# gyuhyun-lee/offline_raytracer

Measured on AMD Instinct MI355X. Metric: Mpaths/s, higher is better.
Workload: dtype f32; 1 GPU; c3_bunny_room.scn (69451 triangles) 1920x1080 1024spp rr0.8, CHUNK policy chunk=64, one frame sharded in 8x8 blocks over 1 GPU(s); width=1920, height=1080, spp=1024, gather=none (1 GPU): un-permute kernel only, gather_fallback=False, launch=single process, workspace_bytes_per_rank=398131200

## Files before the change

offline_raytracer_amd/csrc/ort_device.h:

```cpp
#ifndef ORT_DEVICE_H
#define ORT_DEVICE_H

#include <hip/hip_runtime.h>
#include <stdint.h>

#include "ort_detmath.h"

namespace ortd {

#ifdef ORT_HOST_SIM
#define ORT_D static inline
#else
#define ORT_D __device__ __forceinline__
#endif

struct V3 { float x, y, z; };

constexpr float kPi = 3.14159265358979323846264338327950288419716939937510582097494459230f;
constexpr float kEuler = 2.71828182845904523536028747135266249f;
constexpr float kHitTMin = 0.000001f;
constexpr float kRoughness = 0.01f;
constexpr float kEps = 0.0001f;

ORT_D V3 mk(float x, float y, float z) { V3 r; r.x = x; r.y = y; r.z = z; return r; }
ORT_D V3 add(V3 a, V3 b) { return mk(a.x + b.x, a.y + b.y, a.z + b.z); }
ORT_D V3 sub(V3 a, V3 b) { return mk(a.x - b.x, a.y - b.y, a.z - b.z); }
ORT_D V3 neg(V3 a) { return mk(-a.x, -a.y, -a.z); }
ORT_D V3 scale(float s, V3 a) { return mk(s * a.x, s * a.y, s * a.z); }
ORT_D V3 divs(V3 a, float s) { return mk(a.x / s, a.y / s, a.z / s); }
ORT_D V3 had(V3 a, V3 b) { return mk(a.x * b.x, a.y * b.y, a.z * b.z); }
ORT_D float dot(V3 a, V3 b) { return a.x * b.x + a.y * b.y + a.z * b.z; }
ORT_D float len2(V3 a) { return a.x * a.x + a.y * a.y + a.z * a.z; }
ORT_D float len(V3 a) { return __builtin_sqrtf(a.x * a.x + a.y * a.y + a.z * a.z); }
ORT_D V3 cross(V3 a, V3 b) {
    return mk(a.y * b.z - b.y * a.z, b.x * a.z - a.x * b.z, a.x * b.y - b.x * a.y);
}
ORT_D float absr(float v) { if (v <= 0.0f) v *= -1.0f; return v; }
ORT_D float sq(float v) { return v * v; }
ORT_D bool ceq(float a, float b) { float d = a - b; return d >= -0.000001f && d < 0.000001f; }
ORT_D float sgn(float a) { return (a >= 0.0f) ? 1.0f : -1.0f; }
ORT_D float rmin(float a, float b) { return (a < b) ? a : b; }
ORT_D float rmax(float a, float b) { return (a > b) ? a : b; }
ORT_D V3 normalize(V3 a) {
    float l = len(a);
    if (__builtin_expect(!ceq(l, 0.0f), 1)) return divs(a, l);
    return mk(0, 0, 0);
}
ORT_D bool isnan3(V3 v) { return (v.x != v.x) || (v.y != v.y) || (v.z != v.z); }
ORT_D bool isinf1(float v) { return (om_f32_bits(v) & 0x7fffffffu) == 0x7f800000u; }
ORT_D bool isinf3(V3 v) { return isinf1(v.x) || isinf1(v.y) || isinf1(v.z); }

ORT_D void rng_step(uint32_t &s) { s ^= s << 13; s ^= s >> 17; s ^= s >> 5; }
ORT_D float rng_01(uint32_t &s) { rng_step(s); return (float)s / 4294967296.0f; }
ORT_D float rng_between(uint32_t &s, float lo, float hi) { rng_step(s); return lo + (hi - lo) * rng_01(s); }

ORT_D uint32_t fmix32(uint32_t h) {
    h ^= h >> 16; h *= 0x85ebca6bu; h ^= h >> 13; h *= 0xc2b2ae35u; h ^= h >> 16;
    return h;
}
ORT_D uint32_t job_seed(uint32_t master, uint32_t job) {
    uint32_t h = fmix32(master ^ (job * 2654435761u));
    return h ? h : 1u;
}

struct Mat {
    V3 kd; float ior;
    V3 ks; uint32_t is_light;
    V3 kt; float pd_c;
    V3 emit; float ps_c;
    V3 ed; float pt_c;
};
ORT_D Mat load_mat(const float4 *mats, uint32_t index) {
    const float4 *p = mats + 5u * index;
    float4 a = p[0], b = p[1], c = p[2], d = p[3], e = p[4];
    Mat m;
    m.kd = mk(a.x, a.y, a.z); m.ior = a.w;
    m.ks = mk(b.x, b.y, b.z); m.is_light = om_f32_bits(b.w);
    m.kt = mk(c.x, c.y, c.z); m.pd_c = c.w;
    m.emit = mk(d.x, d.y, d.z); m.ps_c = d.w;
    m.ed = mk(e.x, e.y, e.z); m.pt_c = e.w;
    return m;
}
ORT_D Mat make_mat(V3 kd, V3 ks, V3 kt, float ior) {
    Mat m;
    m.kd = kd; m.ks = ks; m.kt = kt; m.ior = ior; m.is_light = 0; m.emit = mk(0, 0, 0);
    float a = len(kd), b = len(ks), c = len(kt);
    float s = a + b + c;
    m.pd_c = a / s; m.ps_c = b / s; m.pt_c = c / s;
    m.ed = divs(kd, kPi);
// ... 102 lines not shown
        float r = radicand(m, wo, bn.n);
        if (r >= 0.0f) {
            float n_m = dot(N, m), wi_m = dot(wi, m), wo_m = dot(wo, m);
            float denom = sq(bn.no * wo_m + bn.no * wo_m);
            if (!ceq(denom, 0.0f)) {
                float D = ggx_d(N, m, rough);
                pt = D * absr(n_m) * sq(bn.no) * absr(wi_m) / denom;
            }
        }
    }
    return pd_c * pd + ps_c * ps + pt_c * pt;
}

ORT_D float pdf_eval_scattering(V3 N, V3 wi, V3 wo, const Mat &mt, float rough, float dist, float rr, V3 &f) {
    const float wi_n = dot(wi, N), wo_n = dot(wo, N);
    const bool has_ks = len2(mt.ks) > 0.0f, has_kt = len2(mt.kt) > 0.0f;
    V3 H = mk(0, 0, 0);
    float wi_h = 0.0f, D_h = 0.0f, ps = 0.0f;
    if (mt.ps_c > 0.0f || has_ks) {
        H = scale(sgn(wi_n), normalize(add(wo, wi)));
        wi_h = dot(wi, H);
        const float denom = (4.0f * absr(wi_h));
        const bool pdf_needs = mt.ps_c > 0.0f && !ceq(denom, 0.0f);
        if (pdf_needs || (has_ks && wi_h > 0.0f)) D_h = ggx_d(N, H, rough);
        if (pdf_needs) ps = D_h * absr(dot(N, H)) / denom;
    }
    Beer bn; bn.ni = bn.no = bn.n = 0.0f;
    V3 m = mk(0, 0, 0);
    float r = -1.0f, D_m = 0.0f, wi_m = 0.0f, wo_m = 0.0f, pt = ps;
    if (mt.pt_c > 0.0f || has_kt) {
        bn = beer(N, wo, mt.ior);
        m = normalize(neg(add(scale(bn.ni, wi), scale(bn.no, wo))));
        r = radicand(m, wo, bn.n);
        if (!(r < 0.0f)) {
            wi_m = dot(wi, m); wo_m = dot(wo, m);
            D_m = ggx_d(N, m, rough);
        }
        if (r >= 0.0f && mt.pt_c > 0.0f) {
            const float denom = sq(bn.no * wo_m + bn.no * wo_m);
            if (!ceq(denom, 0.0f)) pt = D_m * absr(dot(N, m)) * sq(bn.no) * absr(wi_m) / denom;
        }
    }
    const float pd = absr(wi_n) / kPi;
    const float p = (mt.pd_c * pd + mt.ps_c * ps + mt.pt_c * pt) * rr;
    if (!(p > 0.000001f)) return p;
    V3 Es = mk(0, 0, 0), Et = mk(0, 0, 0);
    if (has_ks && wi_h > 0.0f) {
        V3 F = fresnel(mt.ks, wi_h);
        float G = geom(wi, N, H, rough) * geom(wo, N, H, rough);
        Es = scale((D_h * G) / (4.0f * absr(wi_n) * absr(wo_n)), F);
    }
    if (has_kt) {
        V3 At = mk(1, 1, 1);
        if (wo_n < 0) {
            At.x = ort_powf(kEuler, dist * ort_logf(mt.kt.x));
            At.y = ort_powf(kEuler, dist * ort_logf(mt.kt.y));
            At.z = ort_powf(kEuler, dist * ort_logf(mt.kt.z));
        }
        if (r < 0.0f) {
            if (has_ks) Et = had(At, Es);
        } else {
            V3 F = sub(mk(1, 1, 1), fresnel(mt.ks, wi_m));
            float G = geom(wi, N, m, rough) * geom(wo, N, m, rough);
            float denom = (absr(wi_n) * absr(wo_n) * sq(bn.ni * wi_m + bn.no * wo_m));
            if (!ceq(denom, 0.0f)) {
                V3 nom = scale(D_m * G * absr(wi_m) * absr(wo_m) * sq(bn.no), F);
                Et = had(At, divs(nom, denom));
            }
        }
    }
    f = scale(absr(wi_n), add(add(mt.ed, Es), Et));
    return p;
}

ORT_D V3 sample_lobe_n(V3 N, float c, float cos_phi, float sin_phi) {
    float s = __builtin_sqrtf(1.0f - c * c);
    V3 K = mk(s * cos_phi, s * sin_phi, c);
    if (absr(N.z - 1.0f) < 0.0001f) return K;
    if (absr(N.z + 1.0f) < 0.0001f) return mk(K.x, -K.y, -K.z);
    V3 B = normalize(mk(-N.y, N.x, 0));
    V3 C = cross(N, B);
    return add(add(scale(K.x, B), scale(K.y, C)), scale(K.z, N));
}
ORT_D V3 sample_lobe(V3 N, float c, float phi) { return sample_lobe_n(normalize(N), c, ort_cosf(phi), ort_sinf(phi)); }

struct BrdfDraw { float c, phi, choice; };
template <bool DIFFUSE_SCENE = false>
ORT_D BrdfDraw sample_brdf_draw(uint32_t &rng, float rough, const Mat &mt) {
    float e0 = rng_01(rng), e1 = rng_01(rng);
    BrdfDraw d;
    d.choice = rng_01(rng);
    d.phi = 2.0f * kPi * e1;
    const bool diffuse_lobe = d.choice < mt.pd_c;
    if (DIFFUSE_SCENE ? __builtin_expect(diffuse_lobe, 1) : diffuse_lobe) d.c = __builtin_sqrtf(e0);
    else d.c = ort_cosf(ort_atan2f(rough * __builtin_sqrtf(e0), __builtin_sqrtf(1.0f - e0)));
    return d;
}
template <bool NORMALIZED = true, bool DIFFUSE_SCENE = false>
ORT_D V3 sample_brdf_finish(V3 N, V3 Nn, V3 wo, const Mat &mt, BrdfDraw d, float cos_phi, float sin_phi, bool &is_trans) {
    float pd_c = mt.pd_c, ps_c = mt.ps_c;
    V3 wi;
    is_trans = false;
    V3 m = sample_lobe_n(Nn, d.c, cos_phi, sin_phi);
    const bool diffuse_lobe = d.choice < pd_c;
    if (DIFFUSE_SCENE ? __builtin_expect(diffuse_lobe, 1) : diffuse_lobe) {
        wi = m;
    } else {
        bool refract = !(d.choice >= pd_c && d.choice < pd_c + ps_c);
        Beer bn;
        float r = 0.0f;
        if (refract) {
            bn = beer(N, wo, mt.ior);
            r = radicand(m, wo, bn.n);
            refract = !(r < 0.0f);
        }
        if (!refract) {
            wi = sub(scale(2.0f * absr(dot(wo, m)), m), wo);
        } else {
            wi = sub(scale(bn.n * dot(wo, m) - sgn(dot(wo, N)) * __builtin_sqrtf(r), m), scale(bn.n, wo));
            is_trans = true;
        }
    }
    return NORMALIZED ? normalize(wi) : wi;
}
ORT_D V3 sample_brdf(uint32_t &rng, V3 N, V3 wo, float rough, const Mat &mt, bool &is_trans) {
    BrdfDraw d = sample_brdf_draw(rng, rough, mt);
    return sample_brdf_finish(N, normalize(N), wo, mt, d, ort_cosf(d.phi), ort_sinf(d.phi), is_trans);
}

ORT_D float hit_triangle(V3 v0, V3 e1, V3 e2, V3 o, V3 d) {
    V3 pv = cross(d, e2);
    float det = dot(pv, e1);
    if (!(det <= -0.000001f || det >= 0.000001f)) return -1.0f;
    V3 T = sub(o, v0);
    float u = dot(pv, T) / det;
    if (!(u >= 0.0f)) return -1.0f;
    V3 a = cross(T, e1);
    float v = dot(a, d) / det;
    if (!(v >= 0.0f && u + v <= 1.0f)) return -1.0f;
    float t = dot(a, e2) / det;
    if (!(t >= kHitTMin)) return -1.0f;
    return t;
}

ORT_D float hit_sphere(V3 c, float rad, V3 o, V3 d, V3 &n, bool &tangent) {
    float ht = -1.0f;
    tangent = false;
    V3 rel = sub(o, c);
    float a = dot(d, d), b = dot(d, rel), cc = dot(rel, rel) - rad * rad;
    float root = b * b - a * cc;
    const float tol = 0.00001f;
    if (root >= tol) {
        float sr = __builtin_sqrtf(root);
        float tn = (-b - sr) / a, tp = (-b + sr) / a;
        float t = (tn < 0.0f) ? tp : tn;
        if (t > kHitTMin) {
            ht = t;
            n = scale(1.0f, sub(add(o, scale(ht, d)), c));
        }
    } else if (__builtin_expect(root < tol && root > -tol, 0)) {
        float t = (-b) / (2 * a);
        if (t > kHitTMin) {
            ht = t;
            n = sub(add(o, scale(ht, d)), c);
            tangent = true;
        }
    }
    return ht;
}

ORT_D float hit_aab(V3 lo, V3 hi, V3 o, V3 inv, V3 &n) {
    float ht = -1.0f;
    V3 t0 = had(sub(lo, o), inv), t1 = had(sub(hi, o), inv);
    V3 tmin = mk(rmin(t0.x, t1.x), rmin(t0.y, t1.y), rmin(t0.z, t1.z));
    V3 tmax = mk(rmax(t0.x, t1.x), rmax(t0.y, t1.y), rmax(t0.z, t1.z));
    float max_of_min = rmax(rmax(tmin.x, tmin.y), tmin.z);
    float min_of_max = rmin(rmin(tmax.x, tmax.y), tmax.z);
    if (min_of_max >= max_of_min) {
        float tx = t0.x, ty = t0.y, tz = t0.z;
        float sx = -1.0f, sy = -1.0f, sz = -1.0f;
        if (tx > t1.x) { tx = t1.x; sx = 1.0f; }
        if (ty > t1.y) { ty = t1.y; sy = 1.0f; }
        if (tz > t1.z) { tz = t1.z; sz = 1.0f; }
        float best = tx;
        V3 bn = mk(sx, 0, 0);
        if (best < ty) { best = ty; bn = mk(0, sy, 0); }
// ... 75 lines not shown
```

offline_raytracer_amd/csrc/ort_kernels.hip:

```cpp
#include <algorithm>
#include <memory>
#include <type_traits>

#include "ort_lane.h"
#include "ort_plan.h"
#include "ort_setup.h"

#ifndef ORT_HOST_SIM
void ort_launch_w5(int diffuse, unsigned int grid, void *stream, const void *sv_bytes, const void *hot_bytes);
void ort_w5_layout(size_t sizes[3]);
void ort_launch_radiance_adaptive(int counters, int diffuse, int tabs, unsigned int grid, void *stream, const void *sv_bytes, const void *hot_bytes);
void ort_adaptive_layout(size_t sizes[3]);
void ort_launch_render_adaptive(int counters, int diffuse, int tabs, unsigned int grid, void *stream, const void *sv_bytes, const void *hot_bytes);
void ort_render_adaptive_layout(size_t sizes[3]);

namespace ort {

using namespace ortd;

static_assert(kPlanBlock == (uint32_t)kBlock && kPlanLdsStack == (uint32_t)kLdsStack && kPlanStashVecs == kStashVecs && kPlanCapL == kCapL &&
              kPlanCapR == kCapR && (int)PLAN_JOBS_EXPLICIT == (int)JOBS_EXPLICIT &&
              (int)PLAN_JOBS_PIXEL == (int)JOBS_PIXEL && (int)PLAN_JOBS_CHUNK == (int)JOBS_CHUNK,
              "ort_plan.h counts with the lane code's limits");

#define ORT_HIP(call)                                                                          \
    do {                                                                                       \
        hipError_t e_ = (call);                                                                \
        if (e_ != hipSuccess) {                                                                \
            *err = std::string(#call) + ": " + hipGetErrorString(e_);                          \
            return ORT_ERR_HIP;                                                                \
        }                                                                                      \
    } while (0)

struct DevBuf {
    void *p = nullptr;
    size_t bytes = 0;
    DevBuf() = default;
    DevBuf(DevBuf &&o) noexcept : p(o.p), bytes(o.bytes) { o.p = nullptr; o.bytes = 0; }
    DevBuf &operator=(DevBuf &&o) noexcept { std::swap(p, o.p); std::swap(bytes, o.bytes); return *this; }
    ~DevBuf() { if (p) (void)hipFree(p); }
    int ensure(size_t need, std::string *err) {
        if (bytes >= need && p) return ORT_OK;
        if (p) ORT_HIP(hipFree(p));
        p = nullptr;
        bytes = 0;
        ORT_HIP(hipMalloc(&p, need ? need : 16));
        bytes = need;
        return ORT_OK;
    }
    template <typename T> T *as() const { return (T *)p; }
};

struct DeviceScene {
    explicit DeviceScene(int device_index) : device(device_index) {}
    ~DeviceScene() {
        (void)hipSetDevice(device);
        if (h_active) (void)hipHostFree(h_active);
        for (hipEvent_t ev : {ev0, ev1, ev_done})
            if (ev) (void)hipEventDestroy(ev);
    }
    const int device;
    Knobs knobs;
    DevBuf nodes, tris, spheres, boxes, cyls, materials;
    DevBuf nodes4;
    DevBuf prim_info;
    uint32_t info_box = 0, info_cyl = 0, info_sphere = 0;
    DevBuf light_is_sphere;
    DevBuf tab;
    DevBuf cold;
    DevBuf rv_dev;
    DevBuf view_tab;
    std::vector<float> view_tab_host;
    uint32_t tab_flags = 0;
    uint32_t light_count = 0;
    bool diffuse_only = false;
    DevBuf ref_nodes, ref_recs, chain_boxes;
    DevBuf tri_order, sphere_order, box_order, cyl_order;
    DevBuf bfs_pool, bfs_locks;
    uint32_t bfs_queue_cap = 0, bfs_queue_count = 0;
    unsigned int max_blocks = 0;
    DevBuf ctrl_buf;
    unsigned long long *ctrl() const { return ctrl_buf.as<unsigned long long>(); }
    DevBuf partial, staging, jobs, states;
    hipEvent_t ev0 = nullptr, ev1 = nullptr;
    hipEvent_t ev_done = nullptr;
    bool inflight = false;
    int cu_count = 0;
    DevBuf stash;
    DevBuf drain;
    DevBuf wf_mem;
    unsigned long long *h_active = nullptr;
    DevBuf prim_src;
    float scene_lo[3] = {0, 0, 0}, scene_hi[3] = {0, 0, 0};
    bool scene_box_known = false;
    DevBuf query_stage[6];
};

int device_count(int *n, std::string *err) {
    int c = 0;
    hipError_t e = hipGetDeviceCount(&c);
    if (e != hipSuccess) { *n = 0; *err = std::string("hipGetDeviceCount: ") + hipGetErrorString(e); return ORT_ERR_NO_DEVICE; }
    *n = c;
    return ORT_OK;
}

template <typename T>
static int upload_vec(const std::vector<T> &v, DevBuf *dst, std::string *err) {
    size_t bytes = v.size() * sizeof(T);
    int rc = dst->ensure(bytes, err);
    if (rc) return rc;
    if (bytes) ORT_HIP(hipMemcpy(dst->p, v.data(), bytes, hipMemcpyHostToDevice));
    return ORT_OK;
}

void device_release(Scene *scene) {
    delete scene->dev;
    scene->dev = nullptr;
}

int device_upload(Scene *scene, int device, std::string *err) {
    int n = 0;
    int rc = device_count(&n, err);
    if (rc != ORT_OK) return rc;
    if (n <= 0) { *err = "no HIP device visible"; return ORT_ERR_NO_DEVICE; }
    if (device < 0 || device >= n) { *err = "device index out of range"; return ORT_ERR_INVALID; }
    device_release(scene);
    ORT_HIP(hipSetDevice(device));
    std::unique_ptr<DeviceScene> owner(new DeviceScene(device));
    DeviceScene *d = owner.get();
    const Tree &t = scene->tree;
    if ((rc = upload_vec(t.nodes, &d->nodes, err))) return rc;
    if (!t.nodes4.empty() && 3u * t.max_depth4 <= (uint32_t)(kLdsStack - 4 + kSpillStack))
        if ((rc = upload_vec(t.nodes4, &d->nodes4, err))) return rc;
    if ((rc = upload_vec(t.tris, &d->tris, err))) return rc;
    if ((rc = upload_vec(t.spheres, &d->spheres, err))) return rc;
    if ((rc = upload_vec(t.boxes, &d->boxes, err))) return rc;
    if ((rc = upload_vec(t.cyls, &d->cyls, err))) return rc;
    {
        std::vector<PrimInfo> info;
        build_prim_info(t, scene->ref, info, d->info_box, d->info_cyl, d->info_sphere);
        if ((rc = upload_vec(info, &d->prim_info, err))) return rc;
    }
    const std::vector<DevMaterial> mats = dev_materials(*scene);
    if ((rc = upload_vec(mats, &d->materials, err))) return rc;
    d->diffuse_only = true;
    for (size_t i = 1; i < mats.size(); ++i) {
        const DevMaterial &dm = mats[i];
        if (dm.is_light) continue;
        const float ks2 = dm.specular[0] * dm.specular[0] + dm.specular[1] * dm.specular[1] + dm.specular[2] * dm.specular[2];
        const float kt2 = dm.transmission[0] * dm.transmission[0] + dm.transmission[1] * dm.transmission[1] + dm.transmission[2] * dm.transmission[2];
        if (ks2 > 0.0f || kt2 > 0.0f || dm.ps_c > 0.0f || dm.pt_c > 0.0f) d->diffuse_only = false;
    }
    const std::vector<uint32_t> lis = light_sphere_flags(*scene);
    d->light_count = (uint32_t)lis.size();
    if ((rc = upload_vec(lis, &d->light_is_sphere, err))) return rc;
    {
        std::vector<F4> tab;
        d->tab_flags = pack_lds_tables(t, mats, lis, tab);
        if ((rc = upload_vec(tab, &d->tab, err))) return rc;
    }
    const RefTree &rt = scene->ref;
    if ((rc = upload_vec(rt.nodes, &d->ref_nodes, err))) return rc;
    if ((rc = upload_vec(rt.recs, &d->ref_recs, err))) return rc;
    if ((rc = upload_vec(rt.chain_boxes, &d->chain_boxes, err))) return rc;
    if ((rc = upload_vec(rt.tri_order, &d->tri_order, err))) return rc;
    if ((rc = upload_vec(rt.sphere_order, &d->sphere_order, err))) return rc;
    if ((rc = upload_vec(rt.box_order, &d->box_order, err))) return rc;
    if ((rc = upload_vec(rt.cyl_order, &d->cyl_order, err))) return rc;
    if ((rc = d->ctrl_buf.ensure(128 * sizeof(unsigned long long), err))) return rc;
    ORT_HIP(hipMemset(d->ctrl(), 0, 128 * sizeof(unsigned long long)));
    ORT_HIP(hipEventCreate(&d->ev0));
    ORT_HIP(hipEventCreate(&d->ev1));
    ORT_HIP(hipEventCreateWithFlags(&d->ev_done, hipEventDisableTiming));
    hipDeviceProp_t prop;
    ORT_HIP(hipGetDeviceProperties(&prop, device));
    d->cu_count = prop.multiProcessorCount;
    d->knobs = read_knobs();
    d->max_blocks = upload_max_blocks(d->cu_count, d->knobs);
    d->bfs_queue_cap = (uint32_t)rt.nodes.size() + 8u;
    size_t fit = kBfsPoolBytes / ((size_t)d->bfs_queue_cap * sizeof(uint32_t));
    d->bfs_queue_count = (uint32_t)(fit < 16 ? 16 : (fit > kBfsPoolQueues ? kBfsPoolQueues : fit));
    if ((rc = d->bfs_pool.ensure((size_t)d->bfs_queue_count * d->bfs_queue_cap * sizeof(uint32_t), err))) return rc;
    if ((rc = d->bfs_locks.ensure((size_t)d->bfs_queue_count * kBfsLockStride * sizeof(uint32_t), err))) return rc;
    ORT_HIP(hipMemset(d->bfs_locks.p, 0, d->bfs_locks.bytes));
    ORT_HIP(hipHostMalloc((void **)&d->h_active, sizeof(unsigned long long)));
    {
        SceneCold cold{};
        cold.ref_nodes = d->ref_nodes.as<const float4>(); cold.ref_recs = d->ref_recs.as<const uint32_t>();
        cold.tri_order = d->tri_order.as<const uint32_t>(); cold.sphere_order = d->sphere_order.as<const uint32_t>();
        cold.box_order = d->box_order.as<const uint32_t>(); cold.cyl_order = d->cyl_order.as<const uint32_t>();
        cold.bfs_pool = d->bfs_pool.as<uint32_t>(); cold.bfs_locks = d->bfs_locks.as<uint32_t>();
        cold.bfs_queue_cap = d->bfs_queue_cap; cold.bfs_queue_count = d->bfs_queue_count;
        cold.fallback_counters = d->ctrl() + 6;
        if ((rc = d->rv_dev.ensure(sizeof(RenderView), err))) return rc;
        if ((rc = d->cold.ensure(sizeof(SceneCold), err))) return rc;
        ORT_HIP(hipMemcpy(d->cold.p, &cold, sizeof(SceneCold), hipMemcpyHostToDevice));
    }
    scene->dev = owner.release();
    return ORT_OK;
}

int device_unit_eval(int device, const void *records, uint32_t n, float *out, std::string *err) {
    int count = 0;
    int rc = device_count(&count, err);
    if (rc != ORT_OK) return rc;
    if (device < 0 || device >= count) { *err = "no such HIP device"; return ORT_ERR_NO_DEVICE; }
    ORT_HIP(hipSetDevice(device));
    DevBuf d_rec, d_out;
    if ((rc = d_rec.ensure((size_t)n * 100u + 16, err)) || (rc = d_out.ensure((size_t)n * 32u + 16, err))) return rc;
    ORT_HIP(hipMemcpy(d_rec.p, records, (size_t)n * 100u, hipMemcpyHostToDevice));
    if (n) hipLaunchKernelGGL(unit_eval, dim3((n + 63) / 64), dim3(64), 0, 0, d_rec.as<const uint32_t>(), n, d_out.as<float>());
    ORT_HIP(hipGetLastError());
    ORT_HIP(hipMemcpy(out, d_out.p, (size_t)n * 32u, hipMemcpyDeviceToHost));
    return ORT_OK;
}

template <bool COUNTERS>
static int launch_wavefront(DeviceScene *d, const LaunchPlan &, const SceneView &sv, const RenderView &rvf, const RenderHot &rv, hipStream_t stream, std::string *err) {
    const uint32_t kMaxSlots = 1u << 21;
    unsigned long long want = rvf.job_count < kMaxSlots ? rvf.job_count : kMaxSlots;
    uint32_t S = (uint32_t)((want + kBlock - 1) / kBlock) * kBlock;
    if (S == 0) S = kBlock;
    const size_t per_slot = 16 + 8 + 16 + 4 + 16 + 16 + 16 + 16 + 4;
    size_t need = (size_t)S * per_slot + 4096;
    int rc = d->wf_mem.ensure(need, err);
    if (rc) return rc;
    WfView wf{};
    wf.slots = S;
    char *base = d->wf_mem.as<char>();
    auto carve = [&](size_t bytes) { char *p = base; base += (bytes + 255) & ~(size_t)255; return p; };
    wf.active = (unsigned long long *)carve(256);
    wf.od0 = (float4 *)carve((size_t)S * 16); wf.hit0 = (float4 *)carve((size_t)S * 16);
    wf.p0 = (float4 *)carve((size_t)S * 16); wf.p1 = (float4 *)carve((size_t)S * 16); wf.p2 = (float4 *)carve((size_t)S * 16);
    wf.p3 = (uint4 *)carve((size_t)S * 16);
    wf.od1 = (float2 *)carve((size_t)S * 8);
    wf.hitp = (uint32_t *)carve((size_t)S * 4); wf.flags = (uint32_t *)carve((size_t)S * 4);
    if ((size_t)(base - d->wf_mem.as<char>()) > d->wf_mem.bytes) { *err = "internal: wavefront state carve overflow"; return ORT_ERR_INVALID; }

    unsigned int blocks = S / kBlock;
    unsigned int grid = blocks < d->max_blocks * 2u ? blocks : d->max_blocks * 2u;
    hipLaunchKernelGGL(wf_init, dim3(blocks), dim3(kBlock), 0, stream, wf);
    ORT_HIP(hipGetLastError());
    const int batch = 32;
    for (;;) {
        for (int it = 0; it < batch; ++it) {
            int last = (it == batch - 1);
            if (last) ORT_HIP(hipMemsetAsync(wf.active, 0, sizeof(unsigned long long), stream));
            hipLaunchKernelGGL(wf_shade<COUNTERS>, dim3(grid), dim3(kBlock), 0, stream, sv, rv, wf, last);
            hipLaunchKernelGGL(wf_trace<COUNTERS>, dim3(grid), dim3(kBlock), 0, stream, sv, rv, wf);
        }
        ORT_HIP(hipGetLastError());
        ORT_HIP(hipMemcpyAsync(d->h_active, wf.active, sizeof(unsigned long long), hipMemcpyDeviceToHost, stream));
        ORT_HIP(hipStreamSynchronize(stream));
        if (*d->h_active == 0ull) break;
    }
    return ORT_OK;
}

static int launch_five_waves(DeviceScene *, const LaunchPlan &pl, const SceneView &sv, const RenderView &, const RenderHot &hot, hipStream_t stream, std::string *) {
    ort_launch_w5(pl.diffuse ? 1 : 0, pl.grid, (void *)stream, &sv, &hot);
// ... 25 lines not shown
    loop<true, false, false>(), loop<true, false, true>(), loop<true, true, false>(), loop<true, true, true>(),
    loop<false, false, true, true, true>(), loop<false, true, true, true, true>(), loop<true, false, true, false, true>(),
    views<false, false, false>(), views<false, false, true, true>(), views<false, true, false>(), views<false, true, true, true>(),
    views<true, false, false>(), views<true, false, true>(),
    exchange<false, false>(), exchange<false, true>(), exchange<true, true>(),
    five(false), five(true),
    adaptive(false, false, false), adaptive(false, false, true), adaptive(false, true, false), adaptive(false, true, true),
    adaptive(true, false, false), adaptive(true, false, true), adaptive(true, true, false), adaptive(true, true, true),
};
constexpr bool launchers_match(size_t i = 0) { return i == kBuiltKernelCount || (kLaunchers[i].variant == kBuiltKernels[i] && launchers_match(i + 1)); }
static_assert(sizeof(kLaunchers) / sizeof(kLaunchers[0]) == kBuiltKernelCount && launchers_match(),
              "kLaunchers holds the entries of kBuiltKernels (ort_plan.h), all of them, in its order");

static int launch_path_tracer(DeviceScene *d, const LaunchPlan &pl, const SceneView &sv, const RenderView &rv, const RenderHot &hot, hipStream_t stream, std::string *err) {
    const size_t i = built_index(plan_variant(pl));
    if (i == kBuiltKernelCount) { *err = "internal: no kernel is built for this launch plan"; return ORT_ERR_INTERNAL; }
    if (kLaunchers[i].host) return kLaunchers[i].host(d, pl, sv, rv, hot, stream, err);
    hipLaunchKernelGGL(kLaunchers[i].kernel, dim3(pl.grid), dim3(kBlock), 0, stream, sv, hot);
    return ORT_OK;
}

static int settle_inflight(DeviceScene *d, std::string *err, const char *what = "the previous render on this scene overflowed a reference-order fallback queue") {
    if (!d->inflight) return ORT_OK;
    ORT_HIP(hipEventSynchronize(d->ev_done));
    d->inflight = false;
    unsigned long long ovf = 0;
    ORT_HIP(hipMemcpy(&ovf, d->ctrl() + 7, sizeof(ovf), hipMemcpyDeviceToHost));
    if (ovf) { *err = what; return ORT_ERR_UNSUPPORTED; }
    return ORT_OK;
}

static int reset_ctrl(DeviceScene *d, RenderView *rv, hipStream_t stream, std::string *err) {
    rv->next_job = d->ctrl();
    rv->counters = d->ctrl() + 1;
    ORT_HIP(hipMemsetAsync(d->ctrl(), 0, 128 * sizeof(unsigned long long), stream));
    return ORT_OK;
}
static int upload_view(DeviceScene *d, const RenderView &rv, bool timed, hipStream_t stream, RenderHot *hot, std::string *err) {
    ORT_HIP(hipMemcpyAsync(d->rv_dev.p, &rv, sizeof(RenderView), hipMemcpyHostToDevice, stream));
    *hot = render_hot<RenderHot>(rv, d->rv_dev.p);
    if (timed) ORT_HIP(hipEventRecord(d->ev0, stream));
    return ORT_OK;
}
static int end_kernels(DeviceScene *d, bool timed, hipStream_t stream, std::string *err) {
    ORT_HIP(hipGetLastError());
    if (timed) ORT_HIP(hipEventRecord(d->ev1, stream));
    return ORT_OK;
}
static int mark_inflight(DeviceScene *d, hipStream_t stream, std::string *err) {
    ORT_HIP(hipEventRecord(d->ev_done, stream));
    d->inflight = true;
    return ORT_OK;
}

static int add_launch_stats(const DeviceScene *d, bool counters, bool paths, ort_stats *stats, std::string *err) {
    float ms = 0;
    ORT_HIP(hipEventElapsedTime(&ms, d->ev0, d->ev1));
    unsigned long long c[6];
    ORT_HIP(hipMemcpy(c, d->ctrl() + 1, sizeof(c), hipMemcpyDeviceToHost));
    stats->kernel_ms += ms;
    stats->fallback_rays += c[5];
    if (counters) { stats->rays += c[1]; stats->node_tests += c[2]; stats->tri_tests += c[3]; stats->analytic_tests += c[4]; }
    if (counters && paths) stats->paths += c[0];
    return ORT_OK;
}

static SceneView scene_view(Scene *scene, DeviceScene *d) {
    SceneView sv{};
    sv.nodes = d->nodes.as<const float4>(); sv.tris = d->tris.as<const float4>();
    sv.spheres = d->spheres.as<const float4>(); sv.boxes = d->boxes.as<const float4>(); sv.cyls = d->cyls.as<const float4>();
    sv.prim_info = d->prim_info.as<const PrimInfo>();
    sv.info_box = d->info_box; sv.info_cyl = d->info_cyl; sv.info_sphere = d->info_sphere;
    sv.materials = d->materials.as<const float4>();
    sv.light_is_sphere = d->light_is_sphere.as<const uint32_t>();
    sv.tab_src = d->tab.as<const float4>();
    sv.tab_flags = d->tab_flags;
    sv.light_count = d->light_count;
    sv.pro_boxes = scene->tree.pro_boxes;
    sv.pro_spheres = scene->tree.pro_spheres;
    sv.pro_cyls = scene->tree.pro_cyls;
    sv.chain_boxes = d->chain_boxes.as<const float4>();
    if (getenv("ORT_KNOBS_LIVE")) { const int keep = d->knobs.blocks_per_cu; d->knobs = read_knobs(); d->knobs.blocks_per_cu = keep; }
    sv.force_fallback_mask = d->knobs.force_fallback_mask;
    sv.cold = (const ORT_CONSTANT_AS SceneCold *)d->cold.p;
    return sv;
}

static size_t fast_tree_bytes(const Scene *scene) { return scene->tree.nodes.size() * sizeof(DevNode) + scene->tree.tris.size() * sizeof(DevTri); }

static SceneTraits scene_traits(const Scene *scene, const DeviceScene *d) {
    SceneTraits t;
    t.diffuse_only = d->diffuse_only;
    t.tab_flags = d->tab_flags;
    t.fast_tree_bytes = fast_tree_bytes(scene);
    t.sah_cost = scene->tree.sah_cost;
    t.has_wide = d->nodes4.p != nullptr;
    t.cu_count = d->cu_count;
    t.max_blocks = d->max_blocks;
    return t;
}

static int print_fallback_diag(const DeviceScene *d, const LaunchPlan &pl, std::string *err) {
    unsigned long long fb[2], dg[3];
    ORT_HIP(hipMemcpy(fb, d->ctrl() + 6, sizeof(fb), hipMemcpyDeviceToHost));
    ORT_HIP(hipMemcpy(dg, d->ctrl() + 6 + kDiagFallback, sizeof(dg), hipMemcpyDeviceToHost));
    fprintf(stderr, "fallback: %llu rays traversed again without their first winner, %llu re-cast exactly (%llu octree nodes enqueued, %llu busy queues met)\n",
            dg[1], fb[0], dg[0], dg[2]);
    fprintf(stderr, "issue order: %s\n", pl.block_major ? "block-major" : "chunk-major");
    return ORT_OK;
}

static int print_drain_diag(const DeviceScene *d, const LaunchPlan &pl, std::string *err) {
    std::vector<unsigned long long> t((size_t)pl.grid * (kBlock / 64));
    ORT_HIP(hipMemcpy(t.data(), d->drain.p, t.size() * sizeof(unsigned long long), hipMemcpyDeviceToHost));
    unsigned long long last = 0;
    for (unsigned long long v : t) last = v > last ? v : last;
    const double tick_ms = 1e-5;
    const double marks[] = {0.25, 0.5, 1, 2, 3, 5, 8, 12, 20};
    fprintf(stderr, "drain: of %zu waves, still running before the end of the launch:", t.size());
    for (double m : marks) {
        size_t n = 0;
        for (unsigned long long v : t) n += (double)(last - v) * tick_ms < m ? 1 : 0;
        fprintf(stderr, "  %g ms: %zu", m, n);
    }
    fprintf(stderr, "\n");
    return ORT_OK;
}

static int print_util_diag(const DeviceScene *d, std::string *err) {
    static const char *names[8] = {"node visit", "leaf visit", "traverse outer iteration", "shade call", "  of which lanes with a finished ray",
                                   "produce_ray pass", "  bounce draw", "  sin/cos + ray setup"};
    unsigned long long u[16];
    ORT_HIP(hipMemcpy(u, d->ctrl() + 8, sizeof(u), hipMemcpyDeviceToHost));
    for (int k = 0; k < 8; ++k)
        fprintf(stderr, "util %-40s wave-events %14llu  mean active lanes %6.2f\n", names[k], u[2 * k],
                u[2 * k] ? (double)u[2 * k + 1] / (double)u[2 * k] : 0.0);
    static const char *pnames[10] = {"resolve_hit (chain check)", "hit processing + bounce draw", "pixel / job / new sample", "sin/cos + normalise + ray setup",
                                    "1/d + analytic prologue", "descend loop", "leaf", "pt_lane loop top (after traverse)",
                                    "produce_ray entry (after resolve)", "traverse loop top"};
    unsigned long long ph[30];
    ORT_HIP(hipMemcpy(ph, d->ctrl() + 8 + 32, sizeof(ph), hipMemcpyDeviceToHost));
    double total = 0;
    for (int k = 0; k < 10; ++k) total += (double)ph[3 * k];
    for (int k = 0; k < 10; ++k)
        fprintf(stderr, "phase %-36s share %5.1f %%  cycles/mark %8.1f  marks %12llu  lanes at mark %5.1f\n", pnames[k],
                total > 0 ? 100.0 * (double)ph[3 * k] / total : 0.0, ph[3 * k + 1] ? (double)ph[3 * k] / (double)ph[3 * k + 1] : 0.0,
                ph[3 * k + 1], ph[3 * k + 1] ? (double)ph[3 * k + 2] / (double)ph[3 * k + 1] : 0.0);
    return ORT_OK;
}

static bool same_layout(void (*unit_layout)(size_t *)) {
    size_t s[3];
    unit_layout(s);
    return s[0] == sizeof(SceneView) && s[1] == sizeof(RenderHot) && s[2] == sizeof(RenderView);
}

int device_render(Scene *scene, const ort_render_params *p, const RenderCall &c, void *out_rgb, void *out_spp, void *out_m2, void *states, std::string *err) {
    DeviceScene *d = scene->dev;
    if (!d) { *err = "scene is not uploaded to a device (ort_scene_upload)"; return ORT_ERR_NO_DEVICE; }
    ORT_HIP(hipSetDevice(d->device));
    if (c.ad && !same_layout(ort_render_adaptive_layout)) { *err = "internal: the adaptive render kernels were built with other argument layouts"; return ORT_ERR_INTERNAL; }
    hipStream_t stream = (hipStream_t)c.stream;
    const uint32_t view_count = c.views ? c.view_count : 1u;
    int rc;
    if ((rc = settle_inflight(d, err))) return rc;

// ... 252 lines not shown
```

offline_raytracer_amd/csrc/ort_lane.h:

```cpp
#ifndef ORT_LANE_H
#define ORT_LANE_H

#include <hip/hip_runtime.h>

#include <math.h>
#include <stdio.h>
#include <stdlib.h>
#include <string.h>

#include <algorithm>
#include <string>
#include <vector>

#include "ort_device.h"
#include "ort_scene.h"
#include "ort_setup.h"

#ifdef ORT_W5_TU
#define ORT_NS ort_w5
#elif defined(ORT_ADAPTIVE_TU)
#define ORT_NS ort_ad
#elif defined(ORT_RENDER_ADAPTIVE_TU)
#define ORT_NS ort_ra
#else
#define ORT_NS ort
#endif

namespace ORT_NS {

using namespace ort;
using namespace ortd;

constexpr int kBlock = 256;
#ifndef ORT_LDS_STACK
#define ORT_LDS_STACK 24
#endif
constexpr int kLdsStack = ORT_LDS_STACK;
#ifndef ORT_SPILL_STACK
#define ORT_SPILL_STACK 40
#endif
constexpr int kSpillStack = ORT_SPILL_STACK;
static_assert(kLdsStack - 4 + kSpillStack >= (int)kTreeDepthBudget, "the re-traversal of resolve_hit must hold a tree of kTreeDepthBudget levels");
constexpr uint32_t kBfsPoolQueues = 1024;
constexpr size_t kBfsPoolBytes = 1024u << 20;
constexpr int kDiagFallback = 106;
constexpr uint32_t kBfsLockStride = 32;


#ifdef ORT_HOST_SIM
#define ORT_CONSTANT_AS
#else
#define ORT_CONSTANT_AS __attribute__((address_space(4)))
#endif
struct SceneCold {
    const float4 *ref_nodes;
    const uint32_t *ref_recs;
    const uint32_t *tri_order, *sphere_order, *box_order, *cyl_order;
    uint32_t *bfs_pool;
    uint32_t *bfs_locks;
    uint32_t bfs_queue_cap, bfs_queue_count;
    unsigned long long *fallback_counters;
};

struct PrimInfo { uint32_t chain, mat; };

struct SceneView {
    const float4 *tab_src;
    uint32_t tab_flags;
    const float4 *nodes;
    const float4 *tris;
    const float4 *spheres;
    const float4 *boxes;
    const float4 *cyls;
    const PrimInfo *prim_info;
    uint32_t info_box, info_cyl, info_sphere;
    const float4 *materials;
    const uint32_t *light_is_sphere;
    uint32_t light_count;
    uint32_t pro_boxes, pro_spheres, pro_cyls;
    float cam[12];
    const float4 *chain_boxes;
    const ORT_CONSTANT_AS SceneCold *cold;
    unsigned long long *util;
    uint32_t force_fallback_mask;
};

inline void build_prim_info(const Tree &t, const RefTree &rt, std::vector<PrimInfo> &out, uint32_t &info_box, uint32_t &info_cyl, uint32_t &info_sphere) {
    info_box = (uint32_t)t.tri_mat.size();
    info_cyl = info_box + (uint32_t)t.box_mat.size();
    info_sphere = info_cyl + (uint32_t)t.cyl_mat.size();
    out.assign((size_t)info_sphere + t.sphere_mat.size(), PrimInfo{0u, 0u});
    auto fill = [&out](uint32_t base, const std::vector<uint32_t> &chain, const std::vector<uint32_t> &mat) {
        for (size_t i = 0; i < mat.size(); ++i) out[base + i] = PrimInfo{i < chain.size() ? chain[i] : 0u, mat[i]};
    };
    fill(0u, rt.tri_chain, t.tri_mat);
    fill(info_box, rt.box_chain, t.box_mat);
    fill(info_cyl, rt.cyl_chain, t.cyl_mat);
    fill(info_sphere, rt.sphere_chain, t.sphere_mat);
}

enum : int { JOBS_EXPLICIT = 0, JOBS_PIXEL = 1, JOBS_CHUNK = 2 };

struct RenderView {
    int mode;
    const ort_tile_job *jobs;
    uint32_t *final_states;
    unsigned long long job_count;
    int W, H, x0, y0, x1, y1;
    uint32_t seed, spp, chunk, nchunks;
    float rr;
    int refill_below;
    int descend_below;
    uint32_t shard_index, shard_count, blocks_w, my_blocks;
    uint32_t block_x0, block_y0;
    float *out;
    float *partial;
    int packed_out;
    unsigned long long *next_job;
    unsigned long long *counters;
    float4 *stash;
    uint32_t stash_wave_f4;
    uint32_t capL, capR;
    uint32_t long_min;
    uint32_t long_refill;
    uint32_t park_min;
    uint32_t inflight_cap;
    uint32_t block_major;
    unsigned long long endgame_from;
    uint32_t job_batch;
    unsigned long long batch_until;
    unsigned long long *drain;
    const float4 *views;
    unsigned long long view_jobs;
    uint32_t view_count;
    const float2 *rays;
    const uint32_t *seeds;
    uint32_t ray_tree_spheres, ray_tree_quadrics, ray_tree_boxes;
    float ray_lo[3], ray_hi[3];
    uint32_t ad_min_spp, ad_check_every;
    float ad_tolerance, ad_floor;
    uint32_t *ad_spp;
    float *ad_m2;
};


struct RenderHot {
    int mode, W, H;
    float rr;
    int refill_below, descend_below;
    const ORT_CONSTANT_AS RenderView *c;
};

struct WfView {
    uint32_t slots;
    float4 *od0;
    float2 *od1;
    float4 *hit0;
    uint32_t *hitp;
    float4 *p0;
    float4 *p1;
    float4 *p2;
    uint4 *p3;
    uint32_t *flags;
    unsigned long long *active;
};

enum : int { PS_NEED_JOB = 0, PS_PIXEL = 1, PS_SAMPLE = 2, PS_HIT = 3, PS_DONE = 4 };

#ifdef ORT_HOST_SIM
#define ORT_BALLOT(p) ((p) ? 1ull : 0ull)
#define ORT_POPC64(m) __builtin_popcountll(m)
#define ORT_NEXT_JOB(p) __atomic_fetch_add((p), 1ull, __ATOMIC_RELAXED)
#define ORT_COUNT(p, v) ((void)__atomic_fetch_add((p), (v), __ATOMIC_RELAXED))
#define ORT_TRY_LOCK(p) (*(p) == 0u ? (*(p) = 1u, true) : false)
#define ORT_PEEK(p) (*(p))
#define ORT_BACKOFF()
#define ORT_UNLOCK(p) (*(p) = 0u)
#define ORT_FENCE()
#define ORT_FFS64(m) __builtin_ffsll((long long)(m))
#define ORT_LANE() 0
#define ORT_UTIL(sv, k, pred)
// ... 45 lines not shown
    } while (0)
#endif

#ifndef ORT_HOST_SIM
__shared__ unsigned long long g_lds_prof[96 + 4];
#endif

struct Prof { unsigned long long t = 0; bool on = false; };

#ifndef ORT_DESCEND_SHIFT
#define ORT_DESCEND_SHIFT 2
#endif

#define ORT_RARE(x) __builtin_expect(!!(x), 0)
#if defined(ORT_HOST_SIM) && defined(ORT_CHAIN_STATS)
extern unsigned long long g_cs[4][16];
#define ORT_STAT(row, col) (g_cs[row][col]++)
#else
#define ORT_STAT(row, col) ((void)0)
#endif
constexpr uint32_t kNoPrim = 0xffffffffu;
constexpr uint32_t kTraversalDone = 0xffffffffu;

ORT_D uint32_t prim_order(const SceneView &sv, uint32_t kind, uint32_t slot) {
    return (kind == PRIM_TRI) ? sv.cold->tri_order[slot] : (kind == PRIM_SPHERE) ? sv.cold->sphere_order[slot]
         : (kind == PRIM_BOX) ? sv.cold->box_order[slot] : sv.cold->cyl_order[slot];
}

template <bool COUNTERS, bool EXACT_ORDER, bool FINITE_RAY = false, bool FROM_TAB = false>
ORT_D void test_prim(const SceneView &sv, uint32_t kind, uint32_t slot, V3 org, V3 dir, V3 inv_d, float &best_t, V3 &hit_n,
                     uint32_t &hit_prim, float &phantom_t, float &runner_t, unsigned long long &c_tris, unsigned long long &c_analytic,
                     uint32_t excl = 0xffffffffu, const float4 *rec = nullptr ) {
    float t;
    V3 n = mk(0, 0, 0);
    bool tangent = false;
    if (!EXACT_ORDER && ((kind << 28) | slot) == excl) return;
    if (kind == PRIM_TRI) {
        const float4 *tp = sv.tris + 3u * slot;
        float4 a = tp[0], b = tp[1], c = tp[2];
        if (COUNTERS) c_tris++;
        t = hit_triangle(mk(a.x, a.y, a.z), mk(a.w, b.x, b.y), mk(b.z, b.w, c.x), org, dir);
        n = mk(c.y, c.z, c.w);
    } else if (kind == PRIM_SPHERE) {
        float4 s;
        if (FROM_TAB) s = rec[0]; else s = sv.spheres[slot];
        if (COUNTERS) c_analytic++;
        t = hit_sphere(mk(s.x, s.y, s.z), s.w, org, dir, n, tangent);
    } else if (kind == PRIM_BOX) {
        float4 lo, hi;
        if (FROM_TAB) { lo = rec[0]; hi = rec[1]; } else { lo = sv.boxes[2u * slot]; hi = sv.boxes[2u * slot + 1u]; }
        if (COUNTERS) c_analytic++;
        t = FINITE_RAY ? hit_aab_finite(mk(lo.x, lo.y, lo.z), mk(hi.x, hi.y, hi.z), org, inv_d, n)
                       : hit_aab(mk(lo.x, lo.y, lo.z), mk(hi.x, hi.y, hi.z), org, inv_d, n);
    } else {
        float4 a, b, c, d;
        if (FROM_TAB) { a = rec[0]; b = rec[1]; c = rec[2]; d = rec[3]; }
        else { const float4 *cp = sv.cyls + 4u * slot; a = cp[0]; b = cp[1]; c = cp[2]; d = cp[3]; }
        if (COUNTERS) c_analytic++;
        t = hit_cylinder(mk(a.x, a.y, a.z), a.w, mk(b.x, b.y, b.z), mk(b.w, c.x, c.y), mk(c.z, c.w, d.x), d.y, org, dir, n);
    }
    if (!EXACT_ORDER && tangent) {
        phantom_t = fminf(phantom_t, t);
        return;
    }
    bool take = (t >= kHitTMin && t < best_t);
    if (!EXACT_ORDER && t == best_t && t >= kHitTMin && hit_prim != kNoPrim) {
        take = prim_order(sv, kind, slot) < prim_order(sv, hit_prim >> 28, hit_prim & 0x00ffffffu);
    }
    if (!EXACT_ORDER && t >= kHitTMin) runner_t = fminf(runner_t, take ? best_t : t);
    if (take) {
        best_t = t;
        hit_n = n;
        hit_prim = (kind << 28) | slot;
    }
}

enum : int { CH_ADMIT = 0, CH_REJECT = 1, CH_UNKNOWN = 2 };

ORT_D uint32_t info_index(const SceneView &sv, uint32_t prim) {
    const uint32_t kind = prim >> 28, slot = prim & 0x00ffffffu;
    return slot + ((kind == PRIM_TRI) ? 0u : (kind == PRIM_BOX) ? sv.info_box : (kind == PRIM_CYL) ? sv.info_cyl : sv.info_sphere);
}

template <int BLOCK>
ORT_D void announce_winner(const SceneView &sv, uint32_t prim, uint32_t *lds_stack, int tid) {
    if (prim == kNoPrim) return;
    const PrimInfo *p = sv.prim_info + info_index(sv, prim);
#ifdef ORT_HOST_SIM
    lds_stack[tid] = p->chain;
    lds_stack[BLOCK + tid] = p->mat;
#else
    const uint32_t dst = (uint32_t)__builtin_amdgcn_readfirstlane((int)(uint32_t)(uintptr_t)(lds_stack + (tid & ~63)));
    const uint32_t *q = &p->mat;
    unsigned keep;
    asm volatile("s_mov_b32 %0, m0\n\ts_mov_b32 m0, %3\n\ts_nop 0\n\tglobal_load_lds_dword %1, off\n\t"
                 "s_add_u32 m0, %3, %4\n\ts_nop 0\n\tglobal_load_lds_dword %2, off\n\ts_mov_b32 m0, %0"
                 : "=&s"(keep) : "v"(p), "v"(q), "s"(dst), "n"(BLOCK * 4) : "scc");
#endif
}

template <int BLOCK>
ORT_D void announced_info(const uint32_t *lds_stack, int tid, uint32_t &chain, uint32_t &mat) {
#ifndef ORT_HOST_SIM
    asm volatile("s_waitcnt vmcnt(0)" ::: "memory");
#endif
    chain = lds_stack[tid];
    mat = lds_stack[BLOCK + tid];
}
ORT_D int ref_node_verdict(V3 lo, V3 hi, V3 org, V3 inv_d, float t_hit, float t_other, float &gap) {
    if ((org.x >= lo.x && org.x < hi.x) && (org.y >= lo.y && org.y < hi.y) && (org.z >= lo.z && org.z < hi.z)) return CH_ADMIT;
    const float t = hit_aab_t(lo, hi, org, inv_d);
    if (!(t >= kHitTMin)) return CH_REJECT;
    if (t <= t_hit || (t < t_other && t < t_hit * 1.0001f)) return CH_ADMIT;
    gap = fmaxf(gap, t);
    return CH_UNKNOWN;
}

ORT_D int chain_verdict_full(const SceneView &sv, uint32_t first, uint32_t len, V3 org, V3 inv_d, float t_hit, float t_other, float &gap) {
    int verdict = CH_ADMIT;
    for (uint32_t base = 0; base < len; base += 4u) {
        float4 lo[4], hi[4];
#pragma unroll
        for (uint32_t k = 0; k < 4u; ++k) {
            uint32_t i = base + k;
            i = (i < len) ? i : (len - 1u);
            lo[k] = sv.chain_boxes[2u * (first + i)];
            hi[k] = sv.chain_boxes[2u * (first + i) + 1u];
        }
#pragma unroll
        for (uint32_t k = 0; k < 4u; ++k) {
            const int v = ref_node_verdict(mk(lo[k].x, lo[k].y, lo[k].z), mk(hi[k].x, hi[k].y, hi[k].z), org, inv_d, t_hit, t_other, gap);
            verdict = (v == CH_REJECT || verdict == CH_REJECT) ? CH_REJECT : (v == CH_UNKNOWN ? CH_UNKNOWN : verdict);
        }
        if (verdict == CH_REJECT) break;
    }
    return verdict;
}

ORT_D bool in_rect_half_open(float4 lo, float4 hi, V3 org) {
    return (org.x >= lo.x && org.x < hi.x) && (org.y >= lo.y && org.y < hi.y) && (org.z >= lo.z && org.z < hi.z);
}

constexpr uint32_t kChainNested = 0x08000000u;
#if defined(ORT_HOST_SIM) && defined(ORT_CHAIN_CROSSCHECK)
static unsigned long long g_chain_crosschecks = 0;
#endif
ORT_D int chain_verdict(const SceneView &sv, uint32_t word, V3 org, V3 inv_d, float t_hit, float t_other, float &gap) {
#ifdef ORT_MEASURE_NO_CHAIN
    gap = 0.0f;
    return CH_ADMIT;
#endif
    const uint32_t len = word >> 28, first = word & 0x07ffffffu;
    gap = 0.0f;
    if (len == 0u) return CH_ADMIT;
    const bool finite = (om_f32_bits(inv_d.x) & 0x7fffffffu) < 0x7f800000u && (om_f32_bits(inv_d.y) & 0x7fffffffu) < 0x7f800000u &&
                        (om_f32_bits(inv_d.z) & 0x7fffffffu) < 0x7f800000u;
    if (ORT_RARE(!(word & kChainNested) || !finite)) return chain_verdict_full(sv, first, len, org, inv_d, t_hit, t_other, gap);
    const float4 dlo = sv.chain_boxes[2u * first], dhi = sv.chain_boxes[2u * first + 1u];
    float4 jlo = dlo, jhi = dhi;
    bool found = false;
#ifndef ORT_CHAIN_ROUND
#define ORT_CHAIN_ROUND 2
#endif
    if (len >= 2u) {
        const uint32_t it = len - 1u, it1 = (len >= 3u) ? len - 2u : 1u;
        const float4 plo = sv.chain_boxes[2u * (first + 1u)], phi = sv.chain_boxes[2u * (first + 1u) + 1u];
        const float4 tlo = sv.chain_boxes[2u * (first + it)], thi = sv.chain_boxes[2u * (first + it) + 1u];
        const float4 ulo = sv.chain_boxes[2u * (first + it1)], uhi = sv.chain_boxes[2u * (first + it1) + 1u];
        if (!in_rect_half_open(plo, phi, org)) {
            found = true;
            if (!in_rect_half_open(tlo, thi, org)) { jlo = tlo; jhi = thi; }
            else if (!in_rect_half_open(ulo, uhi, org)) { jlo = ulo; jhi = uhi; }
            else {
                jlo = plo; jhi = phi;
                bool hit = false;
                for (int32_t top = (int32_t)len - 3; ORT_RARE(!hit && top >= 2); top -= ORT_CHAIN_ROUND) {
                    float4 lo[ORT_CHAIN_ROUND], hi[ORT_CHAIN_ROUND];
#pragma unroll
                    for (int32_t k = 0; k < ORT_CHAIN_ROUND; ++k) {
                        int32_t i = top - k;
                        i = (i > 2) ? i : 2;
                        lo[k] = sv.chain_boxes[2u * (first + (uint32_t)i)];
                        hi[k] = sv.chain_boxes[2u * (first + (uint32_t)i) + 1u];
                    }
#pragma unroll
                    for (int32_t k = 0; k < ORT_CHAIN_ROUND; ++k) {
                        const bool outside = !in_rect_half_open(lo[k], hi[k], org);
                        if (!hit && outside) { jlo = lo[k]; jhi = hi[k]; hit = true; }
                    }
                }
            }
        }
    }
#if defined(ORT_HOST_SIM) && defined(ORT_CHAIN_STATS)
    { int jj = -1; for (int32_t i = (int32_t)len - 1; i >= 1; --i) if (!in_rect_half_open(sv.chain_boxes[2u*(first+i)], sv.chain_boxes[2u*(first+i)+1u], org)) { jj = (int)len - 1 - i; break; }
      g_cs[0][len]++; g_cs[1][jj < 0 ? 15 : jj]++; }
#endif
    int verdict = CH_ADMIT;
    if (found && !(hit_aab_t(mk(jlo.x, jlo.y, jlo.z), mk(jhi.x, jhi.y, jhi.z), org, inv_d) >= kHitTMin)) verdict = CH_REJECT;
    else verdict = ref_node_verdict(mk(dlo.x, dlo.y, dlo.z), mk(dhi.x, dhi.y, dhi.z), org, inv_d, t_hit, t_other, gap);
#if defined(ORT_HOST_SIM) && defined(ORT_CHAIN_CROSSCHECK)
    {
        float g2 = 0.0f;
        if (verdict != chain_verdict_full(sv, first, len, org, inv_d, t_hit, t_other, g2)) { fprintf(stderr, "chain shortcut disagrees with the full walk\n"); abort(); }
        g_chain_crosschecks++;
    }
#endif
    return verdict;
}

template <bool COUNTERS>
ORT_D bool ref_raycast_bfs(const SceneView &sv, V3 org, V3 dir, V3 inv_d, uint32_t *queue, float &best_t, V3 &hit_n,
                           uint32_t &hit_prim, unsigned long long &c_nodes, unsigned long long &c_tris,
                           unsigned long long &c_analytic) {
    best_t = 3.402823466e+38f;
    hit_n = mk(0, 0, 0);
    hit_prim = kNoPrim;
    float unused = 0;
    uint32_t head = 0, tail = 0;
    bool ok = true;
    const uint32_t cap = sv.cold->bfs_queue_cap;
    queue[tail++] = 0;
    while (head != tail) {
        uint32_t node = queue[head++];
        const float4 *np = sv.cold->ref_nodes + 3u * node;
        float4 a = np[0], b = np[1], c = np[2];
        int32_t first_child = (int32_t)om_f32_bits(a.w);
        uint32_t rec_first = om_f32_bits(b.w), rec_count = om_f32_bits(c.x);
        for (uint32_t r = 0; r < rec_count; ++r) {
            uint32_t rec = sv.cold->ref_recs[rec_first + r];
            test_prim<COUNTERS, true>(sv, rec >> 28, rec & 0x00ffffffu, org, dir, inv_d, best_t, hit_n, hit_prim, unused, unused, c_tris, c_analytic);
        }
        if (first_child >= 0) {
            for (uint32_t k = 0; k < 8u; ++k) {
                uint32_t ci = (uint32_t)first_child + k;
                const float4 *cp = sv.cold->ref_nodes + 3u * ci;
                float4 ca = cp[0], cb = cp[1], cc = cp[2];
                uint32_t flags = om_f32_bits(cc.y);
                bool leaf_with_records = (flags & 3u) == 3u;
                bool has_children = (int32_t)om_f32_bits(ca.w) >= 0;
                if (!(leaf_with_records || has_children)) continue;
                V3 lo = mk(ca.x, ca.y, ca.z), hi = mk(cb.x, cb.y, cb.z);
                bool add = (org.x >= lo.x && org.x < hi.x) && (org.y >= lo.y && org.y < hi.y) && (org.z >= lo.z && org.z < hi.z);
                if (!add) {
                    float t = hit_aab_t(lo, hi, org, inv_d);
                    if (COUNTERS) c_nodes++;
                    add = (t >= kHitTMin && t < best_t);
                }
                if (add) {
                    if (tail >= cap) { ok = false; continue; }
                    queue[tail++] = ci;
                }
            }
        }
    }
    ORT_COUNT(sv.cold->fallback_counters + kDiagFallback, (unsigned long long)tail);
    return ok;
}

struct Counters {
    unsigned long long paths = 0, rays = 0, nodes = 0, tris = 0, analytic = 0;
};

struct PathState {
    int ps = PS_NEED_JOB;
    uint32_t rng = 0, job_index = 0;
    uint32_t pxy = 0;
    uint32_t jxx = 0;
    uint32_t jyp = 0;
    uint32_t spp = 0, sample = 0;
    V3 color, org, dir, wo, weight;
    bool primary = true;
};

struct AdaptState {
    float q = 0;
    uint32_t next = 0;
};

struct HitState {
    float best_t = 0;
    V3 hit_n;
    uint32_t hit_prim = kNoPrim;
    float phantom_t = 0;
    float runner_t = 0;
    uint32_t hit_mat = 0;
};

ORT_D size_t packed_index(const RenderHot &rv, uint32_t x, uint32_t y) {
    const uint32_t blk = ((y >> 3) - rv.c->block_y0) * rv.c->blocks_w + ((x >> 3) - rv.c->block_x0);
    return (size_t)((blk - rv.c->shard_index) / rv.c->shard_count) * 64u + ((y & 7u) << 3) + (x & 7u);
}
ORT_D float *pixel_ptr(const RenderHot &rv, uint32_t plane, uint32_t x, uint32_t y) {
    if (rv.mode == JOBS_CHUNK) return rv.c->partial + ((size_t)plane * rv.c->my_blocks * 64u + packed_index(rv, x, y)) * 3u;
    if (rv.c->packed_out) return rv.c->out + packed_index(rv, x, y) * 3u;
    return rv.c->out + 3u * ((size_t)y * (size_t)rv.W + (size_t)x);
}

ORT_D float *view_pixel_ptr(const RenderHot &rv, uint32_t view, uint32_t plane, uint32_t x, uint32_t y) {
    if (rv.mode == JOBS_CHUNK) return rv.c->partial + (((size_t)view * rv.c->nchunks + plane) * rv.c->my_blocks * 64u + packed_index(rv, x, y)) * 3u;
    return rv.c->out + 3u * (((size_t)view * (size_t)rv.H + (size_t)y) * (size_t)rv.W + (size_t)x);
}

struct Trav {
    uint32_t cur = 0;
    int sp = 0;
    V3 inv_d;
};

ORT_D void reset_hit(HitState &h, float best_t) {
    h.best_t = best_t;
    h.hit_n = mk(0, 0, 0);
    h.hit_prim = kNoPrim;
    h.phantom_t = __builtin_inff();
    h.runner_t = __builtin_inff();
}

template <bool COUNTERS, bool TABS, bool HAS_EXCL = false>
ORT_D void prologue_tests(const SceneView &sv, const float4 *tab, V3 org, V3 dir, V3 inv_d, HitState &h, Counters &c, uint32_t excl = kNoPrim) {
    const float4 *pb = nullptr, *ps = nullptr, *pc = nullptr;
    if (TABS) { pb = tab + kTabPro; ps = pb + 2u * sv.pro_boxes; pc = ps + sv.pro_spheres; }
#ifndef ORT_PROLOGUE_DEFER
#define ORT_PROLOGUE_DEFER 1
#endif
    if (!ORT_PROLOGUE_DEFER && ORT_BALLOT(!all_finite6(org, inv_d)) == 0ull) {
        for (uint32_t i = 0; i < sv.pro_boxes; ++i)
            test_prim<COUNTERS, false, true, TABS>(sv, PRIM_BOX, i, org, dir, inv_d, h.best_t, h.hit_n, h.hit_prim, h.phantom_t, h.runner_t, c.tris, c.analytic, excl, TABS ? pb + 2u * i : nullptr);
    } else
    if (ORT_BALLOT(!all_finite6(org, inv_d)) == 0ull) {
        for (uint32_t i = 0; i < sv.pro_boxes; ++i) {
            float4 lo, hi;
            if (TABS) { lo = pb[2u * i]; hi = pb[2u * i + 1u]; } else { lo = sv.boxes[2u * i]; hi = sv.boxes[2u * i + 1u]; }
            const uint32_t prim = ((uint32_t)PRIM_BOX << 28) | i;
            if (COUNTERS && (!HAS_EXCL || prim != excl)) c.analytic++;
            float t = hit_aab_t_finite(mk(lo.x, lo.y, lo.z), mk(hi.x, hi.y, hi.z), org, inv_d);
            if (HAS_EXCL && ORT_RARE(prim == excl)) t = -1.0f;
            bool take = (t >= kHitTMin && t < h.best_t);
            if (ORT_RARE(t == h.best_t && t >= kHitTMin && h.hit_prim != kNoPrim))
                take = prim_order(sv, PRIM_BOX, i) < prim_order(sv, h.hit_prim >> 28, h.hit_prim & 0x00ffffffu);
            if (t >= kHitTMin) h.runner_t = fminf(h.runner_t, take ? h.best_t : t);
            if (take) { h.best_t = t; h.hit_prim = prim; }
        }
        if ((h.hit_prim >> 28) == PRIM_BOX && h.hit_prim != kNoPrim) {
            const uint32_t i = h.hit_prim & 0x00ffffffu;
            float4 lo, hi;
            if (TABS) { lo = pb[2u * i]; hi = pb[2u * i + 1u]; } else { lo = sv.boxes[2u * i]; hi = sv.boxes[2u * i + 1u]; }
            V3 n = mk(0, 0, 0);
            (void)hit_aab_finite(mk(lo.x, lo.y, lo.z), mk(hi.x, hi.y, hi.z), org, inv_d, n);
            h.hit_n = n;
        }
    } else {
        for (uint32_t i = 0; i < sv.pro_boxes; ++i)
            test_prim<COUNTERS, false, false, TABS>(sv, PRIM_BOX, i, org, dir, inv_d, h.best_t, h.hit_n, h.hit_prim, h.phantom_t, h.runner_t, c.tris, c.analytic, excl, TABS ? pb + 2u * i : nullptr);
    }
    for (uint32_t i = 0; i < sv.pro_spheres; ++i)
        test_prim<COUNTERS, false, false, TABS>(sv, PRIM_SPHERE, i, org, dir, inv_d, h.best_t, h.hit_n, h.hit_prim, h.phantom_t, h.runner_t, c.tris, c.analytic, excl, TABS ? ps + i : nullptr);
    for (uint32_t i = 0; i < sv.pro_cyls; ++i)
        test_prim<COUNTERS, false, false, TABS>(sv, PRIM_CYL, i, org, dir, inv_d, h.best_t, h.hit_n, h.hit_prim, h.phantom_t, h.runner_t, c.tris, c.analytic, excl, TABS ? pc + 4u * i : nullptr);
}

#ifndef ORT_HOST_SIM
ORT_D float wave_bcast(float v, int lane) { return om_bits_f32((uint32_t)__builtin_amdgcn_readlane((int)om_f32_bits(v), lane)); }
ORT_D uint32_t wave_bcast(uint32_t v, int lane) { return (uint32_t)__builtin_amdgcn_readlane((int)v, lane); }
ORT_D uint32_t rank_in(unsigned long long mask) {
    return __builtin_amdgcn_mbcnt_hi((uint32_t)(mask >> 32), __builtin_amdgcn_mbcnt_lo((uint32_t)mask, 0u));
}

template <bool COUNTERS>
ORT_D bool ref_raycast_bfs_wave(const SceneView &sv, const int leader, V3 org_l, V3 dir_l, V3 inv_l, uint32_t *queue, float &out_t, V3 &out_n,
                                uint32_t &out_prim, unsigned long long &c_nodes, unsigned long long &c_tris, unsigned long long &c_analytic) {
// ... 121 lines not shown
        const bool ok = ref_raycast_bfs_wave<COUNTERS>(sv, leader, org, dir, inv_d, sv.cold->bfs_pool + (size_t)slot * sv.cold->bfs_queue_cap, h.best_t, h.hit_n,
                                                       h.hit_prim, c.nodes, c.tris, c.analytic);
#endif
        ORT_FENCE();
        if (ORT_LANE() == leader) {
            if (!ok) ORT_COUNT(sv.cold->fallback_counters + 1, 1ull);
            ORT_UNLOCK(sv.cold->bfs_locks + slot * kBfsLockStride);
        }
        pending &= pending - 1ull;
    }
}

ORT_D V3 focal_point(const RenderHot &rv, uint32_t pxy, V3 cam_p, V3 cam_x, V3 cam_y, V3 cam_z, float focal_length) {
    float fx = (2.0f * (int)(pxy & 0xffffu) / (float)rv.W) - 1.0f;
    float fy = (2.0f * (int)(pxy >> 16) / (float)rv.H) - 1.0f;
    V3 to_pixel = normalize(sub(add(scale(fx, cam_x), scale(fy, cam_y)), cam_z));
    return add(cam_p, scale(focal_length, to_pixel));
}

struct ViewCamera { V3 p, x, y, z; };
ORT_D ViewCamera load_view_camera(const RenderHot &rv, uint32_t v) {
    const float4 *q = rv.c->views + 4u * (size_t)v;
    const float4 a = q[0], b = q[1], c = q[2], d = q[3];
    ViewCamera cam;
    cam.p = mk(a.x, a.y, a.z);
    cam.x = mk(b.x, b.y, b.z);
    cam.y = mk(c.x, c.y, c.z);
    cam.z = mk(d.x, d.y, d.z);
    return cam;
}
ORT_D V3 view_focal_point(const RenderHot &rv, uint32_t pxy, const ViewCamera &cam) {
    return focal_point(rv, pxy, cam.p, cam.x, cam.y, cam.z, len(sub(cam.p, mk(0, 0, 0.2f))));
}
ORT_D V3 view_aperture_point(const ViewCamera &cam, float aperture, float cs, float sn) {
    return sub(add(add(cam.p, scale(aperture * cs, cam.x)), scale(aperture * sn, cam.y)), scale(0.1f, cam.z));
}

#ifndef ORT_HOST_SIM
ORT_D unsigned long long draw_job(const RenderHot &rv, unsigned long long *pool) {
    const unsigned long long mask = __ballot(true);
    const uint32_t n = (uint32_t)__popcll(mask);
    const uint32_t rank = (uint32_t)__builtin_amdgcn_mbcnt_hi((uint32_t)(mask >> 32), __builtin_amdgcn_mbcnt_lo((uint32_t)mask, 0u));
    const unsigned long long next = ((volatile unsigned long long *)pool)[0], end = ((volatile unsigned long long *)pool)[1];
    const uint32_t avail = (uint32_t)(end - next);
    unsigned long long j = next + rank;
    if (n > avail) {
        const uint32_t need = n - avail;
        uint32_t want = rv.c->job_batch;
        if (want < need || end >= rv.c->batch_until) want = need;
        unsigned long long base = 0ull;
        if (rank == 0u) base = atomicAdd(rv.c->next_job, (unsigned long long)want);
        const uint32_t lo = (uint32_t)__builtin_amdgcn_readfirstlane((int)(uint32_t)base);
        const uint32_t hi = (uint32_t)__builtin_amdgcn_readfirstlane((int)(uint32_t)(base >> 32));
        base = ((unsigned long long)hi << 32) | lo;
        if (rank >= avail) j = base + (rank - avail);
        if (rank == 0u) { ((volatile unsigned long long *)pool)[0] = base + need; ((volatile unsigned long long *)pool)[1] = base + want; }
    } else if (rank == 0u) {
        ((volatile unsigned long long *)pool)[0] = next + n;
    }
    return j;
}
ORT_D unsigned long long *wave_job_pool(const RenderHot &rv, unsigned long long *lds_pool) {
    unsigned long long *pool = lds_pool + 2u * (threadIdx.x >> 6);
    if ((threadIdx.x & 63u) == 0u) { ((volatile unsigned long long *)pool)[0] = 0ull; ((volatile unsigned long long *)pool)[1] = 0ull; }
    return rv.c->job_batch > 1u ? pool : nullptr;
}
#else
ORT_D unsigned long long draw_job(const RenderHot &rv, unsigned long long *) { return ORT_NEXT_JOB(rv.c->next_job); }
#endif

ORT_D float adaptive_luminance(V3 e) { return (0.2126f * e.x + 0.7152f * e.y) + 0.0722f * e.z; }
ORT_D bool adaptive_stop(V3 C, float Q, uint32_t n, float tolerance, float lum_floor) {
    const float fn = (float)n;
    const float m = adaptive_luminance(C) / fn;
    float v = Q / fn - m * m;
    if (v < 0.0f) v = 0.0f;
    const float vm = v / (fn - 1.0f);
    const float a = m < 0.0f ? -m : m;
    const float b = a > lum_floor ? a : lum_floor;
    const float thr = tolerance * b;
    return vm <= thr * thr;
}

template <bool COUNTERS, bool DIFFUSE = false, bool TABS = false, bool IMPLICIT = false, bool VIEWS = false, bool RAYS = false, bool ADAPT = false>
ORT_D bool produce_ray(const SceneView &sv, const RenderHot &rv, const float4 *tab, PathState &P, const HitState &h, Counters &c, Prof &pr,
                       float *focal_cache = nullptr, int focal_stride = 0, uint32_t spp_u = 0, uint32_t *late_flag = nullptr, bool no_new_job = false,
                       unsigned long long *pool = nullptr, AdaptState *A = nullptr) {
    static_assert(!ADAPT || (IMPLICIT && (RAYS || VIEWS)), "the adaptive rule is built for the radiance queries and for one-pixel jobs of a batch of views");
    const V3 cam_p = mk(sv.cam[0], sv.cam[1], sv.cam[2]);
    const V3 cam_x = mk(sv.cam[3], sv.cam[4], sv.cam[5]);
    const V3 cam_y = mk(sv.cam[6], sv.cam[7], sv.cam[8]);
    const V3 cam_z = mk(sv.cam[9], sv.cam[10], sv.cam[11]);
    const float focal_length = len(sub(cam_p, mk(0, 0, 0.2f)));
    const float aperture = 0.1f;

    while (P.ps != PS_DONE) {
        ORT_UTIL(sv, 5, true);
        ORT_PHASE(pr, sv, 8, true);
        bool bounce = false;
        float angle = 0.0f;
        BrdfDraw draw;
        Mat m;
        V3 n, focal;
        V3 ray_o = mk(0, 0, 0), ray_d = mk(0, 0, 0);
        if (P.ps == PS_HIT) {
            bool alive = true;
            const uint32_t hit_mat = h.hit_mat;
            n = normalize(h.hit_n);
            ORT_SIM_RAY_HOOK((int)(P.pxy & 0xffffu), (int)(P.pxy >> 16), P.org, P.dir, h.best_t, n, hit_mat);
            if (COUNTERS && P.primary) c.paths++;
            if (hit_mat) {
                if (TABS) m = load_mat(tab + kTabMats, hit_mat);
                else m = load_mat(sv.materials, hit_mat);
            }
            if (!hit_mat) {
                alive = false;
            } else if (m.is_light) {
                V3 e = P.primary ? m.emit : had(P.weight, m.emit);
                if (P.primary || (!isnan3(e) && !isinf3(e))) {
                    P.color = add(P.color, e);
                    if constexpr (ADAPT) { const float y = adaptive_luminance(e); A->q = A->q + y * y; }
                }
                alive = false;
            } else {
                if (P.primary) {
                    if (len2(m.kd) > 0.0f) P.weight = had(P.weight, m.kd);
                } else {
                    if (DIFFUSE) {
                        float p = pdf_brdf<true>(n, P.dir, P.wo, kRoughness, m) * rv.rr;
                        if (p > 0.000001f) {
                            V3 f = eval_scattering<true>(n, P.dir, P.wo, m, kRoughness, h.best_t);
                            P.weight = had(divs(f, p), P.weight);
                        }
                    } else {
                        V3 f = mk(0, 0, 0);
                        const float p = pdf_eval_scattering(n, P.dir, P.wo, m, kRoughness, h.best_t, rv.rr, f);
                        if (p > 0.000001f) P.weight = had(divs(f, p), P.weight);
                    }
                    P.wo = neg(P.dir);
                }
                P.org = add(P.org, scale(h.best_t - kEps, P.dir));
            }
            P.primary = false;
            bounce = alive && rng_01(P.rng) < rv.rr;
            if (bounce) {
                rng_step(P.rng);
                if (sv.light_count) {
                    uint32_t li = P.rng % sv.light_count;
                    uint32_t is_sphere;
                    if (TABS) is_sphere = ((const uint32_t *)tab)[4 * kTabLights + li];
                    else is_sphere = sv.light_is_sphere[li];
                    if (is_sphere) { rng_step(P.rng); rng_step(P.rng); rng_step(P.rng); rng_step(P.rng); }
                }
                ORT_UTIL(sv, 6, true);
                draw = sample_brdf_draw<DIFFUSE>(P.rng, kRoughness, m);
                angle = draw.phi;
            } else {
                P.sample++;
                P.ps = PS_SAMPLE;
                if constexpr (ADAPT) {
                    if (P.sample == A->next && P.sample < spp_u) {
                        const uint32_t after = A->next + rv.c->ad_check_every;
                        A->next = after < A->next ? 0xffffffffu : after;
                        if (adaptive_stop(P.color, A->q, P.sample, rv.c->ad_tolerance, rv.c->ad_floor)) A->next = 0u;
                    }
                }
            }
            ORT_PHASE(pr, sv, 1, true);
        }
        if (!bounce) {
            const uint32_t job_spp = IMPLICIT ? spp_u : P.spp;
            bool job_ends = P.ps == PS_SAMPLE && P.sample == job_spp;
            if constexpr (ADAPT) job_ends = P.ps == PS_SAMPLE && (P.sample == job_spp || A->next == 0u);
            if (job_ends) {
                V3 o = divs(P.color, (float)(ADAPT ? P.sample : job_spp));
                if constexpr (RAYS) {
                    const size_t ray = ((size_t)P.pxy << 32) | P.job_index;
                    float *p = rv.c->out + 3u * ray;
                    p[0] = o.x; p[1] = o.y; p[2] = o.z;
                    if (rv.c->final_states) rv.c->final_states[ray] = P.rng;
                    if constexpr (ADAPT) {
                        if (rv.c->ad_spp) rv.c->ad_spp[ray] = P.sample;
                        if (rv.c->ad_m2) rv.c->ad_m2[ray] = A->q;
                    }
                    P.ps = PS_NEED_JOB;
                } else {
                uint32_t px = P.pxy & 0xffffu, py = P.pxy >> 16;
                float *p;
                if constexpr (VIEWS) p = view_pixel_ptr(rv, P.job_index, P.jyp >> 16, px, py);
                else p = pixel_ptr(rv, P.jyp >> 16, px, py);
                p[0] = o.x; p[1] = o.y; p[2] = o.z;
                if constexpr (ADAPT) {
                    const size_t at = ((size_t)P.job_index * (size_t)rv.H + (size_t)py) * (size_t)rv.W + (size_t)px;
                    if (rv.c->ad_spp) rv.c->ad_spp[at] = P.sample;
                    if (rv.c->ad_m2) rv.c->ad_m2[at] = A->q;
                    if (rv.c->final_states) rv.c->final_states[at] = P.rng;
                }
                if (IMPLICIT) {
                    P.ps = PS_NEED_JOB;
                } else {
                px++;
                if (px == (P.jxx >> 16)) { px = P.jxx & 0xffffu; py++; }
                P.pxy = px | (py << 16);
                if (py == (P.jyp & 0xffffu)) {
                    if (rv.mode == JOBS_EXPLICIT && rv.c->final_states) rv.c->final_states[P.job_index] = P.rng;
                    P.ps = PS_NEED_JOB;
                } else {
                    P.ps = PS_PIXEL;
                }
                }
                }
            }
            if (P.ps == PS_NEED_JOB) {
                if (no_new_job) return false;
                unsigned long long j;
#ifndef ORT_HOST_SIM
                if (pool) j = draw_job(rv, pool);
                else
#endif
                j = ORT_NEXT_JOB(rv.c->next_job);
                if (j >= rv.c->job_count) { P.ps = PS_DONE; break; }
                if (IMPLICIT && late_flag && j >= rv.c->endgame_from) *late_flag = 1u;
                if constexpr (RAYS) {
                    const float2 *r = rv.c->rays + 3ull * j;
                    const float2 a = r[0], b = r[1], e = r[2];
                    const uint32_t seed = rv.c->seeds[j];
                    const V3 d = mk(b.y, e.x, e.y);
                    const float l2 = len2(d);
                    if (!(all_finite6(mk(a.x, a.y, b.x), d) && l2 >= 0.999f && l2 <= 1.001f)) {
                        float *p = rv.c->out + 3u * (size_t)j;
                        p[0] = p[1] = p[2] = om_bits_f32(0x7fc00000u);
// ... 12 lines not shown
                    ort_tile_job jb = rv.c->jobs[j];
                    P.job_index = (uint32_t)j;
                    P.jxx = (uint32_t)jb.x0 | ((uint32_t)jb.x1 << 16);
                    P.jyp = (uint32_t)jb.y1;
                    P.pxy = (uint32_t)jb.x0 | ((uint32_t)jb.y0 << 16);
                    P.rng = jb.rng_state; P.spp = jb.spp;
                    if (jb.x1 <= jb.x0 || jb.y1 <= jb.y0) {
                        if (rv.c->final_states) rv.c->final_states[P.job_index] = P.rng;
                        continue;
                    }
                } else {
                    uint32_t seed;
                    if constexpr (VIEWS) {
                        P.job_index = (uint32_t)(j / rv.c->view_jobs);
                        j = j % rv.c->view_jobs;
                        seed = om_f32_bits(rv.c->views[4u * (size_t)P.job_index].w);
                    }
                    unsigned long long per_chunk = (unsigned long long)rv.c->my_blocks * 64ull;
                    uint32_t k, lb, pin;
                    if (rv.c->block_major) {
                        const uint32_t per_block = rv.c->nchunks * 64u;
                        const uint32_t within = (uint32_t)(j % per_block);
                        lb = (uint32_t)(j / per_block);
                        k = within >> 6;
                        pin = within & 63u;
                    } else {
                        k = (uint32_t)(j / per_chunk);
                        const uint32_t rem = (uint32_t)(j % per_chunk);
                        lb = rem >> 6;
                        pin = rem & 63u;
                    }
                    uint32_t blk = rv.c->shard_index + lb * rv.c->shard_count;
                    int x = (int)((rv.c->block_x0 + blk % rv.c->blocks_w) * 8u + (pin & 7u));
                    int y = (int)((rv.c->block_y0 + blk / rv.c->blocks_w) * 8u + (pin >> 3));
                    if (x < rv.c->x0 || x >= rv.c->x1 || y < rv.c->y0 || y >= rv.c->y1) continue;
                    uint32_t pix = (uint32_t)(y * rv.W + x);
                    if (!IMPLICIT) P.jxx = (uint32_t)x | ((uint32_t)(x + 1) << 16);
                    P.pxy = (uint32_t)x | ((uint32_t)y << 16);
                    if (rv.mode == JOBS_PIXEL) {
                        if constexpr (VIEWS) P.rng = job_seed(seed, pix);
                        else P.rng = job_seed(rv.c->seed, pix);
                        if (!IMPLICIT) P.spp = rv.c->spp;
                        P.jyp = (uint32_t)(y + 1);
                    } else {
                        if constexpr (VIEWS) P.rng = job_seed(seed, k * (uint32_t)(rv.W * rv.H) + pix);
                        else P.rng = job_seed(rv.c->seed, k * (uint32_t)(rv.W * rv.H) + pix);
                        if (!IMPLICIT) P.spp = rv.c->chunk;
                        P.jyp = (uint32_t)(y + 1) | (k << 16);
                    }
                }
                P.ps = PS_PIXEL;
            }
            if (P.ps == PS_PIXEL) {
                ORT_SIM_PIXEL_HOOK((int)(P.pxy & 0xffffu), (int)(P.pxy >> 16), P.rng);
                P.color = mk(0, 0, 0);
                P.sample = 0;
                P.ps = PS_SAMPLE;
                if constexpr (ADAPT) { A->q = 0.0f; A->next = rv.c->ad_min_spp; }
                if (focal_cache) {
                    V3 f;
                    if constexpr (VIEWS) f = view_focal_point(rv, P.pxy, load_view_camera(rv, P.job_index));
                    else f = focal_point(rv, P.pxy, cam_p, cam_x, cam_y, cam_z, focal_length);
                    focal_cache[0] = f.x; focal_cache[focal_stride] = f.y; focal_cache[2 * focal_stride] = f.z;
                }
            }
            if (P.sample == job_spp) continue;
            if constexpr (RAYS) {
                const float2 *r = rv.c->rays + 3ull * (((unsigned long long)P.pxy << 32) | P.job_index);
                const float2 a = r[0], b = r[1], e = r[2];
                ray_o = mk(a.x, a.y, b.x);
                ray_d = mk(b.y, e.x, e.y);
            } else {
            if constexpr (VIEWS)
                focal = focal_cache ? mk(focal_cache[0], focal_cache[focal_stride], focal_cache[2 * focal_stride])
                                    : view_focal_point(rv, P.pxy, load_view_camera(rv, P.job_index));
            else
            focal = focal_cache ? mk(focal_cache[0], focal_cache[focal_stride], focal_cache[2 * focal_stride])
                                : focal_point(rv, P.pxy, cam_p, cam_x, cam_y, cam_z, focal_length);
            angle = rng_between(P.rng, 0.0f, 2 * kPi);
            }
            ORT_PHASE(pr, sv, 2, true);
        }
        ORT_UTIL(sv, 7, true);
        float cs, sn;
        ort_sincosf(angle, &sn, &cs);
        if (DIFFUSE) {
            V3 ap = mk(0, 0, 0);
            if (!bounce) {
                if constexpr (RAYS) ap = ray_o;
                else
                if constexpr (VIEWS) ap = view_aperture_point(load_view_camera(rv, P.job_index), aperture, cs, sn);
                else
                ap = sub(add(add(cam_p, scale(aperture * cs, cam_x)), scale(aperture * sn, cam_y)), scale(0.1f, cam_z));
            }
            const V3 unit1 = normalize(bounce ? n : (RAYS ? ray_d : sub(focal, ap)));
            bool is_trans = false;
            V3 raw = unit1;
            if (bounce) raw = sample_brdf_finish<false, true>(n, unit1, P.wo, m, draw, cs, sn, is_trans);
            const V3 unit2 = normalize(raw);
            if (bounce) {
                if (is_trans) P.org = add(P.org, scale(2.0f * kEps, P.dir));
                P.dir = unit2;
            } else {
                if constexpr (RAYS) { P.dir = ray_d; P.wo = neg(unit1); }
                else {
                P.dir = unit1;
                P.wo = neg(unit2);
                }
                P.org = ap;
                P.weight = mk(1, 1, 1);
                P.primary = true;
                P.ps = PS_HIT;
            }
        } else {
            V3 raw, ap = mk(0, 0, 0);
            bool is_trans = false;
            if (bounce) {
                raw = sample_brdf_finish<false>(n, normalize(n), P.wo, m, draw, cs, sn, is_trans);
            } else {
                if constexpr (RAYS) ap = ray_o;
                else
                if constexpr (VIEWS) ap = view_aperture_point(load_view_camera(rv, P.job_index), aperture, cs, sn);
                else
                ap = sub(add(add(cam_p, scale(aperture * cs, cam_x)), scale(aperture * sn, cam_y)), scale(0.1f, cam_z));
                if constexpr (RAYS) raw = ray_d;
                else
                raw = sub(focal, ap);
            }
            const V3 unit = normalize(raw);
            if (bounce) {
                if (is_trans) P.org = add(P.org, scale(2.0f * kEps, P.dir));
                P.dir = unit;
            } else {
                if constexpr (RAYS) { P.dir = raw; P.wo = neg(unit); }
                else {
                P.dir = unit;
                P.wo = neg(normalize(P.dir));
                }
                P.org = ap;
                P.weight = mk(1, 1, 1);
                P.primary = true;
                P.ps = PS_HIT;
            }
        }
        ORT_PHASE(pr, sv, 3, true);
        return true;
    }
    return false;
}


constexpr float kCullSlack = 0.9997996f;

template <bool COUNTERS, int LDS_ENTRIES, int BLOCK>
ORT_D void visit_node(float4 a, float4 b, float4 cc, float4 d, V3 org, V3 inv_d, float best_t, uint32_t &cur, int &sp, uint32_t *lds_stack,
                      uint32_t *spill, int tid, Counters &c) {
    uint32_t c0 = om_f32_bits(d.x), c1 = om_f32_bits(d.y);
    if (COUNTERS) c.nodes += 2;
    float t0x = (a.x - org.x) * inv_d.x, t1x = (a.w - org.x) * inv_d.x;
    float t0y = (a.y - org.y) * inv_d.y, t1y = (b.x - org.y) * inv_d.y;
    float t0z = (a.z - org.z) * inv_d.z, t1z = (b.y - org.z) * inv_d.z;
    float n0 = fmaxf(fmaxf(fminf(t0x, t1x), fminf(t0y, t1y)), fminf(t0z, t1z));
    float f0 = fminf(fminf(fmaxf(t0x, t1x), fmaxf(t0y, t1y)), fmaxf(t0z, t1z));
    float u0x = (b.z - org.x) * inv_d.x, u1x = (cc.y - org.x) * inv_d.x;
    float u0y = (b.w - org.y) * inv_d.y, u1y = (cc.z - org.y) * inv_d.y;
    float u0z = (cc.x - org.z) * inv_d.z, u1z = (cc.w - org.z) * inv_d.z;
    float n1 = fmaxf(fmaxf(fminf(u0x, u1x), fminf(u0y, u1y)), fminf(u0z, u1z));
    float f1 = fminf(fminf(fmaxf(u0x, u1x), fmaxf(u0y, u1y)), fmaxf(u0z, u1z));
    bool h0 = (f0 * 1.0000004f >= n0) && (f0 >= 0.0f) && ((n0 * kCullSlack < best_t) || (c0 & SPHERE_BELOW_BIT));
    bool h1 = (f1 * 1.0000004f >= n1) && (f1 >= 0.0f) && ((n1 * kCullSlack < best_t) || (c1 & SPHERE_BELOW_BIT)) && (c1 != EMPTY_CHILD);
    if (h0 && h1) {
        bool swap = n1 < n0;
        uint32_t farc = swap ? c0 : c1;
        cur = swap ? c1 : c0;
        if (sp < LDS_ENTRIES) lds_stack[sp * BLOCK + tid] = farc;
        else spill[sp - LDS_ENTRIES] = farc;
        sp++;
    } else if (h0) {
        cur = c0;
    } else if (h1) {
        cur = c1;
    } else if (sp == 0) {
        cur = kTraversalDone;
    } else {
        sp--;
        if (sp < LDS_ENTRIES) cur = lds_stack[sp * BLOCK + tid];
        else cur = ((volatile uint32_t *)spill)[sp - LDS_ENTRIES];
    }
}

template <bool COUNTERS, int LDS_ENTRIES, int BLOCK>
ORT_D void visit_node4(float4 lx, float4 ly, float4 lz, float4 hx, float4 hy, float4 hz, float4 cw, V3 org, V3 inv_d, float best_t, uint32_t &cur, int &sp,
                       uint32_t *lds_stack, uint32_t *spill, int tid, Counters &c) {
    if (COUNTERS) c.nodes += 4;
    float key0, key1, key2, key3;
    uint32_t w0, w1, w2, w3;
#define ORT_SLAB4(K, W, LX, LY, LZ, HX, HY, HZ, CW)                                                                        \
    {                                                                                                                      \
        const float t0x = ((LX) - org.x) * inv_d.x, t1x = ((HX) - org.x) * inv_d.x;                                        \
        const float t0y = ((LY) - org.y) * inv_d.y, t1y = ((HY) - org.y) * inv_d.y;                                        \
        const float t0z = ((LZ) - org.z) * inv_d.z, t1z = ((HZ) - org.z) * inv_d.z;                                        \
        const float n_ = fmaxf(fmaxf(fminf(t0x, t1x), fminf(t0y, t1y)), fminf(t0z, t1z));                                  \
        const float f_ = fminf(fminf(fmaxf(t0x, t1x), fmaxf(t0y, t1y)), fmaxf(t0z, t1z));                                  \
        const uint32_t cw_ = om_f32_bits(CW);                                                                              \
        const bool hit_ = (f_ * 1.0000004f >= n_) && (f_ >= 0.0f) && ((n_ * kCullSlack < best_t) || (cw_ & SPHERE_BELOW_BIT)) && (cw_ != EMPTY_CHILD); \
        K = hit_ ? fminf(n_, 3.402823466e+38f) : __builtin_inff();              \
        W = hit_ ? cw_ : EMPTY_CHILD;                                                                                      \
    }
    ORT_SLAB4(key0, w0, lx.x, ly.x, lz.x, hx.x, hy.x, hz.x, cw.x)
    ORT_SLAB4(key1, w1, lx.y, ly.y, lz.y, hx.y, hy.y, hz.y, cw.y)
    ORT_SLAB4(key2, w2, lx.z, ly.z, lz.z, hx.z, hy.z, hz.z, cw.z)
    ORT_SLAB4(key3, w3, lx.w, ly.w, lz.w, hx.w, hy.w, hz.w, cw.w)
#undef ORT_SLAB4
#define ORT_CX(KA, WA, KB, WB)                                                                                             \
    {                                                                                                                      \
        const bool sw_ = KB < KA;                                                                                          \
        const float ka_ = sw_ ? KB : KA, kb_ = sw_ ? KA : KB;                                                              \
        const uint32_t wa_ = sw_ ? WB : WA, wb_ = sw_ ? WA : WB;                                                           \
        KA = ka_; KB = kb_; WA = wa_; WB = wb_;                                                                            \
    }
    ORT_CX(key0, w0, key1, w1)
    ORT_CX(key2, w2, key3, w3)
    ORT_CX(key0, w0, key2, w2)
    ORT_CX(key1, w1, key3, w3)
    ORT_CX(key1, w1, key2, w2)
#undef ORT_CX
    if (w0 == EMPTY_CHILD) {
        if (sp == 0) {
            cur = kTraversalDone;
        } else {
            sp--;
            if (sp < LDS_ENTRIES) cur = lds_stack[sp * BLOCK + tid];
            else cur = ((volatile uint32_t *)spill)[sp - LDS_ENTRIES];
        }
        return;
    }
    cur = w0;
    if (w3 != EMPTY_CHILD) { if (sp < LDS_ENTRIES) lds_stack[sp * BLOCK + tid] = w3; else spill[sp - LDS_ENTRIES] = w3; sp++; }
    if (w2 != EMPTY_CHILD) { if (sp < LDS_ENTRIES) lds_stack[sp * BLOCK + tid] = w2; else spill[sp - LDS_ENTRIES] = w2; sp++; }
    if (w1 != EMPTY_CHILD) { if (sp < LDS_ENTRIES) lds_stack[sp * BLOCK + tid] = w1; else spill[sp - LDS_ENTRIES] = w1; sp++; }
}

template <bool COUNTERS, bool TABS, int LDS_ENTRIES, int BLOCK>
ORT_D void begin_ray(const SceneView &sv, const float4 *tab, const PathState &P, Trav &T, HitState &h, Counters &c, Prof &pr,
                     uint32_t *lds_stack, uint32_t *spill, int tid) {
    T.cur = 0;
    T.sp = 0;
    T.inv_d = mk(1.0f / P.dir.x, 1.0f / P.dir.y, 1.0f / P.dir.z);
    reset_hit(h, 3.402823466e+38f);
    prologue_tests<COUNTERS, TABS>(sv, tab, P.org, P.dir, T.inv_d, h, c);
    ORT_PHASE(pr, sv, 4, true);
}

template <bool COUNTERS, int LDS_ENTRIES, int BLOCK, bool TREELET = false, bool ANNOUNCE = false, bool WIDE = false>
ORT_D bool traverse(const SceneView &sv, V3 org, V3 dir, Trav &T, HitState &h, uint32_t *lds_stack, uint32_t *spill, int tid,
                    int refill_below, int descend_below, Counters &c, Prof &pr, uint32_t excl = kNoPrim, const float4 *tab = nullptr) {
    bool tracing = true;
    uint32_t cur = T.cur;
    int sp = T.sp;
    const V3 inv_d = T.inv_d;
    while (tracing) {
        ORT_UTIL(sv, 2, true);
        ORT_PHASE(pr, sv, 9, true);
        const int entering = ORT_POPC64(ORT_BALLOT((cur & LEAF_BIT) == 0u));
        const int stragglers = descend_below < (entering >> ORT_DESCEND_SHIFT) ? descend_below : (entering >> ORT_DESCEND_SHIFT);
        while (!(cur & LEAF_BIT)) {
            ORT_UTIL(sv, 0, true);
            const uint32_t ni = cur & NODE_INDEX_MASK;
            if (WIDE) {
                const float4 *np = sv.nodes + 8u * ni;
                const float4 lx = np[0], ly = np[1], lz = np[2], hx = np[3], hy = np[4], hz = np[5], cw = np[6];
                visit_node4<COUNTERS, LDS_ENTRIES, BLOCK>(lx, ly, lz, hx, hy, hz, cw, org, inv_d, h.best_t, cur, sp, lds_stack, spill, tid, c);
            } else {
            float4 na, nb, nc, nd;
            if (TREELET && ni < kTreeletNodes) {
                const float4 *np = tab + kTabTreelet + 4u * ni;
                na = np[0]; nb = np[1]; nc = np[2]; nd = np[3];
            } else {
                const float4 *np = sv.nodes + 4u * ni;
                na = np[0]; nb = np[1]; nc = np[2]; nd = np[3];
            }
            visit_node<COUNTERS, LDS_ENTRIES, BLOCK>(na, nb, nc, nd, org, inv_d, h.best_t, cur, sp, lds_stack, spill, tid, c);
            }
            if (ORT_POPC64(ORT_BALLOT(true)) < stragglers) break;
        }
        ORT_PHASE(pr, sv, 5, true);
        if (!(cur & LEAF_BIT)) {
        } else if (cur == kTraversalDone) {
            tracing = false;
        } else {
            ORT_UTIL(sv, 1, true);
            uint32_t kind = (cur >> 28) & 7u, count = ((cur >> 24) & 15u) + 1u, first = cur & 0x00ffffffu;
            for (uint32_t i = 0; i < count; ++i)
                test_prim<COUNTERS, false>(sv, kind, first + i, org, dir, inv_d, h.best_t, h.hit_n, h.hit_prim, h.phantom_t, h.runner_t, c.tris, c.analytic, excl);
            if (sp == 0) {
                cur = kTraversalDone;
                tracing = false;
            } else {
                sp--;
                if (sp < LDS_ENTRIES) cur = lds_stack[sp * BLOCK + tid];
                else cur = ((volatile uint32_t *)spill)[sp - LDS_ENTRIES];
            }
            ORT_PHASE(pr, sv, 6, true);
        }
        if (ANNOUNCE && !tracing) announce_winner<BLOCK>(sv, h.hit_prim, lds_stack, tid);
        if (refill_below > 0 && ORT_POPC64(ORT_BALLOT(tracing)) < refill_below) break;
    }
    T.cur = cur;
    T.sp = sp;
    return tracing;
}

template <bool COUNTERS, bool TABS, int LDS_ENTRIES, int BLOCK, bool ANNOUNCED = false, bool WIDE = false>
ORT_D void resolve_hit(const SceneView &sv, const float4 *tab, V3 org, V3 dir, V3 inv_d, uint32_t lane_id, HitState &h, Counters &c, Prof &pr,
                       uint32_t *lds_stack, uint32_t *spill, int tid) {
    uint32_t word = 0, mat = 0;
    if (ANNOUNCED) {
        announced_info<BLOCK>(lds_stack, tid, word, mat);
    } else if (h.hit_prim != kNoPrim) {
        const PrimInfo pi = sv.prim_info[info_index(sv, h.hit_prim)];
        word = pi.chain; mat = pi.mat;
    }
    bool stale = false;
    bool recast = sv.force_fallback_mask != 0xffffffffu && (om_f32_bits(dir.x) & sv.force_fallback_mask) == 0u;
    if (!ORT_RARE(recast)) {
        if (ORT_RARE(h.phantom_t <= h.best_t)) {
            recast = true;
            ORT_STAT(2, 1);
        } else if (h.hit_prim != kNoPrim) {
            float gap = 0.0f;
            const int verdict = chain_verdict(sv, word, org, inv_d, h.best_t, fminf(h.runner_t, h.phantom_t), gap);
            if (ORT_RARE(verdict != CH_ADMIT)) {
                stale = true;
                ORT_STAT(3, verdict == CH_REJECT ? 0 : 1); ORT_STAT(3, 4 + (int)(h.hit_prim >> 28));
                ORT_COUNT(sv.cold->fallback_counters + kDiagFallback + 1, 1ull);
                const uint32_t w_prim = h.hit_prim;
                uint32_t *save = lds_stack + tid;
                save[(LDS_ENTRIES - 1) * BLOCK] = om_f32_bits(h.best_t);
                save[(LDS_ENTRIES - 2) * BLOCK] = om_f32_bits(h.hit_n.x);
                save[(LDS_ENTRIES - 3) * BLOCK] = om_f32_bits(h.hit_n.y);
                save[(LDS_ENTRIES - 4) * BLOCK] = om_f32_bits(h.hit_n.z);
                Trav t2;
                t2.cur = 0; t2.sp = 0; t2.inv_d = inv_d;
                reset_hit(h, verdict == CH_REJECT ? 3.402823466e+38f : om_bits_f32(om_f32_bits(gap) + 1u));
                prologue_tests<COUNTERS, TABS, true>(sv, tab, org, dir, inv_d, h, c, w_prim);
                (void)traverse<COUNTERS, LDS_ENTRIES - 4, BLOCK, false, false, WIDE>(sv, org, dir, t2, h, lds_stack, spill, tid, 0, 0, c, pr, w_prim);
                if (verdict == CH_UNKNOWN) {
                    if (h.hit_prim != kNoPrim || h.phantom_t <= gap) {
                        recast = true;
                        ORT_STAT(2, h.hit_prim != kNoPrim ? 2 : 6);
                    } else {
                        h.best_t = om_bits_f32(save[(LDS_ENTRIES - 1) * BLOCK]);
                        h.hit_n = mk(om_bits_f32(save[(LDS_ENTRIES - 2) * BLOCK]), om_bits_f32(save[(LDS_ENTRIES - 3) * BLOCK]),
                                     om_bits_f32(save[(LDS_ENTRIES - 4) * BLOCK]));
                        h.hit_prim = w_prim;
                    }
                } else if (h.phantom_t <= h.best_t) {
                    recast = true;
                    ORT_STAT(2, 3);
                } else if (h.hit_prim != kNoPrim) {
                    float gap2 = 0.0f;
                    if (chain_verdict(sv, sv.prim_info[info_index(sv, h.hit_prim)].chain, org, inv_d, h.best_t, fminf(h.runner_t, h.phantom_t), gap2) != CH_ADMIT) { recast = true; ORT_STAT(2, 4); }
                }
            }
        }
    }
    recast_exactly<COUNTERS>(sv, recast, org, dir, inv_d, lane_id, h, c);
    if (ORT_RARE(stale || recast)) mat = (h.hit_prim != kNoPrim) ? sv.prim_info[info_index(sv, h.hit_prim)].mat : 0u;
    h.hit_mat = (h.hit_prim != kNoPrim) ? mat : 0u;
}

ORT_D void flush_counters(const RenderHot &rv, const Counters &c, bool all) {
    if (all) {
        ORT_COUNT(rv.c->counters + 0, c.paths);
        ORT_COUNT(rv.c->counters + 1, c.rays);
        ORT_COUNT(rv.c->counters + 2, c.nodes);
        ORT_COUNT(rv.c->counters + 3, c.tris);
        ORT_COUNT(rv.c->counters + 4, c.analytic);
    }
}

template <bool COUNTERS, bool DIFFUSE = false, bool TABS = false, bool IMPLICIT = false, bool WIDE = false, bool VIEWS = false, bool ADAPT = false>
ORT_D void pt_lane(const SceneView &sv, const RenderHot &rv, const float4 *tab, uint32_t *lds_stack, float *lds_focal, const int tid,
                   const uint32_t lane_id, bool prof_on = false, unsigned long long *pool = nullptr, AdaptState *A = nullptr) {
    uint32_t spill[kSpillStack];
    const uint32_t spp_u = IMPLICIT ? ((rv.mode == JOBS_PIXEL) ? rv.c->spp : rv.c->chunk) : 0u;
    Prof pr;
    pr.on = prof_on;
#ifndef ORT_HOST_SIM
    if (COUNTERS && prof_on) pr.t = __builtin_amdgcn_s_memtime();
#endif
    PathState P;
    HitState h;
    Trav T;
    Counters c;
    bool tracing = false;
    for (;;) {
        if (!tracing) {
            ORT_UTIL(sv, 3, true);
            ORT_UTIL(sv, 4, P.ps == PS_HIT);
            ORT_PHASE(pr, sv, 7, true);
            if (P.ps == PS_HIT) resolve_hit<COUNTERS, TABS, kLdsStack, kBlock, true, WIDE>(sv, tab, P.org, P.dir, T.inv_d, lane_id, h, c, pr, lds_stack, spill, tid);
            ORT_PHASE(pr, sv, 0, P.ps == PS_HIT);
            if constexpr (ADAPT) tracing = produce_ray<COUNTERS, DIFFUSE, TABS, IMPLICIT, VIEWS, false, true>(sv, rv, tab, P, h, c, pr, lds_focal + tid, kBlock, spp_u, nullptr, false, pool, A);
            else
            tracing = produce_ray<COUNTERS, DIFFUSE, TABS, IMPLICIT, VIEWS>(sv, rv, tab, P, h, c, pr, lds_focal + tid, kBlock, spp_u, nullptr, false, pool);
            if (tracing) {
                begin_ray<COUNTERS, TABS, kLdsStack, kBlock>(sv, tab, P, T, h, c, pr, lds_stack, spill, tid);
                if (COUNTERS) c.rays++;
            }
        }
        if (ORT_BALLOT(P.ps != PS_DONE) == 0ull) break;
        if (tracing) tracing = traverse<COUNTERS, kLdsStack, kBlock, TABS && !WIDE, true, WIDE>(sv, P.org, P.dir, T, h, lds_stack, spill, tid, rv.refill_below, rv.descend_below, c, pr, kNoPrim, tab);
    }
    flush_counters(rv, c, COUNTERS);
}


#ifndef ORT_HOST_SIM
struct Stash {
    float4 *rec;
    uint32_t *stk;
    uint32_t cap;
};

ORT_D uint32_t lane_rank(unsigned long long mask) {
    return __builtin_amdgcn_mbcnt_hi((uint32_t)(mask >> 32), __builtin_amdgcn_mbcnt_lo((uint32_t)mask, 0u));
}

constexpr uint32_t kStashVecs = 9u;
constexpr uint32_t kCapL = 128u, kCapR = 192u;
static_assert(kLdsStack % 4 == 0, "the L stash carves its stack words out of float4 units (kLdsStack / 4 per parked path)");
ORT_D void stash_store(const Stash &st, uint32_t slot, const PathState &P, const HitState &h, uint32_t cur, int sp, V3 inv_d, const float *focal_cache,
                       uint32_t info_chain = 0u, uint32_t info_mat = 0u) {
    float4 *r = st.rec + slot;
    const uint32_t cap = st.cap;
    r[0] = make_float4(P.org.x, P.org.y, P.org.z, P.dir.x);
    r[cap] = make_float4(P.dir.y, P.dir.z, h.best_t, om_bits_f32(h.hit_prim));
    r[2u * cap] = make_float4(h.hit_n.x, h.hit_n.y, h.hit_n.z, h.phantom_t);
    r[3u * cap] = make_float4(h.runner_t, om_bits_f32(cur), om_bits_f32((uint32_t)sp), om_bits_f32(P.rng));
    r[4u * cap] = make_float4(P.color.x, P.color.y, P.color.z, P.weight.x);
    r[5u * cap] = make_float4(P.weight.y, P.weight.z, P.wo.x, P.wo.y);
    r[6u * cap] = make_float4(P.wo.z, om_bits_f32(P.pxy), om_bits_f32(P.jyp), om_bits_f32(P.sample | (P.primary ? 0x80000000u : 0u)));
    r[7u * cap] = make_float4(inv_d.x, inv_d.y, inv_d.z, focal_cache[0]);
    r[8u * cap] = make_float4(focal_cache[kBlock], focal_cache[2 * kBlock], om_bits_f32(info_chain), om_bits_f32(info_mat));
}

ORT_D void stash_load(const Stash &st, uint32_t slot, const RenderHot &rv, PathState &P, HitState &h, Trav &T, float *focal_cache, uint32_t *lds_info) {
    const float4 *r = st.rec + slot;
    const uint32_t cap = st.cap;
    const float4 a = r[0], b = r[cap], c = r[2u * cap], d = r[3u * cap], e = r[4u * cap], f = r[5u * cap], g = r[6u * cap];
    const float4 i = r[7u * cap], j = r[8u * cap];
    P.org = mk(a.x, a.y, a.z); P.dir = mk(a.w, b.x, b.y);
    h.best_t = b.z; h.hit_prim = om_f32_bits(b.w);
    h.hit_n = mk(c.x, c.y, c.z); h.phantom_t = c.w;
    h.runner_t = d.x; T.cur = om_f32_bits(d.y); T.sp = (int)om_f32_bits(d.z); P.rng = om_f32_bits(d.w);
    P.color = mk(e.x, e.y, e.z); P.weight = mk(e.w, f.x, f.y); P.wo = mk(f.z, f.w, g.x);
    P.pxy = om_f32_bits(g.y); P.jyp = om_f32_bits(g.z);
    const uint32_t sm = om_f32_bits(g.w);
    P.sample = sm & 0x7fffffffu; P.primary = (sm >> 31) != 0u;
    P.ps = PS_HIT;
    T.inv_d = mk(i.x, i.y, i.z);
    focal_cache[0] = i.w; focal_cache[kBlock] = j.x; focal_cache[2 * kBlock] = j.y;
    lds_info[0] = om_f32_bits(j.z); lds_info[kBlock] = om_f32_bits(j.w);
}

template <bool COUNTERS, bool DIFFUSE, bool TABS>
ORT_D void pt_lane_x(const SceneView &sv, const RenderHot &rv, const float4 *tab, uint32_t *lds_stack, float *lds_focal, const int tid,
                     const uint32_t lane_id, bool prof_on, unsigned long long *pool) {
    uint32_t spill[kSpillStack];
    Prof pr;
    pr.on = prof_on;
    if (COUNTERS && prof_on) pr.t = __builtin_amdgcn_s_memtime();
    PathState P;
    HitState h;
    Trav T;
    Counters c;
    bool tracing = false;

    const uint32_t wave = (uint32_t)__builtin_amdgcn_readfirstlane((int)(lane_id >> 6));
    const uint32_t spp_u = (rv.mode == JOBS_PIXEL) ? rv.c->spp : rv.c->chunk;
    float4 *wbase = rv.c->stash + (size_t)wave * rv.c->stash_wave_f4;
    Stash L, R;
    L.rec = wbase; L.cap = kCapL;
    L.stk = (uint32_t *)(wbase + kStashVecs * kCapL);
    R.rec = wbase + (kStashVecs + (uint32_t)kLdsStack / 4u) * kCapL; R.cap = kCapR; R.stk = nullptr;
    uint32_t ltop = 0, rtop = 0;
    float *focal_cache = lds_focal + tid;
    uint32_t *late_flag = (uint32_t *)lds_focal + 3 * kBlock + tid;
    *late_flag = 0u;
    bool early_end = false;

    for (;;) {
        if (!early_end) early_end = __ballot(*(volatile uint32_t *)late_flag != 0u) != 0ull;
        const unsigned long long m_tr = __ballot(tracing);
        const unsigned long long m_done = __ballot(!tracing && P.ps == PS_HIT);
// ... 357 lines not shown
    if (count_active && produced) atomicAdd(wf.active, produced);
    flush_counters(rv, c, COUNTERS);
}

template <bool COUNTERS>
__global__ void __launch_bounds__(kBlock) wf_trace(SceneView sv, RenderHot rv, WfView wf) {
    __shared__ uint32_t lds_stack[kWfLdsStack * kBlock];
    const float4 *lds_tab = nullptr;
    uint32_t spill[kWfSpill];
    Counters c;
    const uint32_t stride = gridDim.x * (uint32_t)kBlock;
    const uint32_t lane_id = blockIdx.x * (uint32_t)kBlock + threadIdx.x;
    for (uint32_t i = lane_id; i < wf.slots; i += stride)
        wf_trace_slot<COUNTERS>(sv, lds_tab, wf, i, lane_id, lds_stack, spill, (int)threadIdx.x, c);
    flush_counters(rv, c, COUNTERS);
}

__global__ void wf_init(WfView wf) {
    uint32_t i = blockIdx.x * blockDim.x + threadIdx.x;
    if (i < wf.slots) wf.flags[i] = (uint32_t)PS_NEED_JOB;
    if (i == 0) *wf.active = 0ull;
}

__global__ void unit_eval(const uint32_t *records, uint32_t n, float *out) {
    uint32_t i = blockIdx.x * blockDim.x + threadIdx.x;
    if (i >= n) return;
    const uint32_t *rec = records + 25u * i;
    float a[24];
    for (int k = 0; k < 24; ++k) a[k] = om_bits_f32(rec[1 + k]);
    float o[8];
    unit_eval_op(rec[0], a, o);
    for (int k = 0; k < 8; ++k) out[8u * i + k] = o[k];
}

__global__ void combine_chunks(RenderHot rv) {
    unsigned long long idx = (unsigned long long)blockIdx.x * blockDim.x + threadIdx.x;
    if (idx >= (unsigned long long)rv.c->my_blocks * 64ull) return;
    combine_pixel(rv, idx);
}
__global__ void combine_chunks_views(RenderHot rv) {
    const unsigned long long idx = (unsigned long long)blockIdx.x * blockDim.x + threadIdx.x, per_view = (unsigned long long)rv.c->my_blocks * 64ull;
    if (idx >= per_view * rv.c->view_count) return;
    combine_pixel(rv, idx % per_view, (uint32_t)(idx / per_view));
}

#endif
#endif

#ifndef ORT_W5_TU
struct RaycastIO {
    const float2 *rays;
    uint2 *hits;
    const uint32_t *prim_src;
    uint32_t tree_spheres;
    uint32_t tree_quadrics;
    uint32_t tree_boxes;
    float lo[3], hi[3];
};

ORT_D bool raycast_needs_exact(const RaycastIO &io, V3 org, V3 dir, V3 inv_d) {
    const bool short_dir = io.tree_quadrics && !(len2(dir) >= (io.tree_spheres ? 0.999f : 1e-30f));
    const bool inv_nonfinite = io.tree_boxes && !(((inv_d.x - inv_d.x) + (inv_d.y - inv_d.y)) + (inv_d.z - inv_d.z) == 0.0f);
    const bool far = io.tree_quadrics && !(org.x >= io.lo[0] && org.x <= io.hi[0] && org.y >= io.lo[1] && org.y <= io.hi[1] &&
                                          org.z >= io.lo[2] && org.z <= io.hi[2]);
    return short_dir || far || inv_nonfinite;
}

template <bool COUNTERS, bool TABS>
ORT_D void raycast_lane(const SceneView &sv, const RenderHot &rv, const RaycastIO &io, const float4 *tab, uint32_t *lds_stack, const int tid,
                        const uint32_t lane_id, unsigned long long *pool) {
    uint32_t spill[kSpillStack];
    PathState P;
    HitState h;
    Trav T;
    Counters c;
    Prof pr;
    unsigned long long ray = 0;
    bool tracing = false, held = false, more = true;
    for (;;) {
        if (!tracing) {
            if (held) {
                resolve_hit<COUNTERS, TABS, kLdsStack, kBlock, true>(sv, tab, P.org, P.dir, T.inv_d, lane_id, h, c, pr, lds_stack, spill, tid);
                const uint32_t src = h.hit_prim != kNoPrim ? io.prim_src[info_index(sv, h.hit_prim)] : kNoPrim;
                const V3 n = normalize(h.hit_n);
                uint2 *o = io.hits + 3ull * ray;
                o[0] = make_uint2(om_f32_bits(h.best_t), om_f32_bits(n.x));
                o[1] = make_uint2(om_f32_bits(n.y), om_f32_bits(n.z));
                o[2] = make_uint2(h.hit_mat, src);
                held = false;
            }
            if (more) {
                const unsigned long long j = pool ? draw_job(rv, pool) : ORT_NEXT_JOB(rv.c->next_job);
                if (j < rv.c->job_count) {
                    const float2 *r = io.rays + 3ull * j;
                    const float2 a = r[0], b = r[1], e = r[2];
                    P.org = mk(a.x, a.y, b.x);
                    P.dir = mk(b.y, e.x, e.y);
                    ray = j;
                    begin_ray<COUNTERS, TABS, kLdsStack, kBlock>(sv, tab, P, T, h, c, pr, lds_stack, spill, tid);
                    if (ORT_RARE(raycast_needs_exact(io, P.org, P.dir, T.inv_d))) {
                        T.cur = kTraversalDone;
                        h.phantom_t = 0.0f;
                    }
                    if (COUNTERS) c.rays++;
                    tracing = held = true;
                } else {
                    more = false;
                }
            }
        }
        if (ORT_BALLOT(tracing) == 0ull) break;
        if (tracing) tracing = traverse<COUNTERS, kLdsStack, kBlock, TABS, true>(sv, P.org, P.dir, T, h, lds_stack, spill, tid, rv.refill_below, rv.descend_below, c, pr, kNoPrim, tab);
    }
    flush_counters(rv, c, COUNTERS);
}

#ifndef ORT_HOST_SIM
template <bool COUNTERS, bool TABS>
__global__ void __launch_bounds__(kBlock) __attribute__((amdgpu_waves_per_eu(ORT_WAVES_PER_EU, ORT_WAVES_PER_EU)))
raycast_rays(SceneView sv, RenderHot rv, RaycastIO io) {
    __shared__ uint32_t lds_stack[kLdsStack * kBlock];
    __shared__ unsigned long long lds_pool[2 * (kBlock / 64)];
    __shared__ float4 lds_tab[TABS ? kTabF4 : 1];
    if (TABS) fill_tab(sv, lds_tab);
    raycast_lane<COUNTERS, TABS>(sv, rv, io, lds_tab, lds_stack, (int)threadIdx.x, blockIdx.x * (uint32_t)kBlock + threadIdx.x, wave_job_pool(rv, lds_pool));
}
#endif

struct OccludedIO {
    RaycastIO q;
    const float *tmax;
    uint8_t *out;
    uint32_t mats_nonzero;
};

template <bool COUNTERS, bool TABS>
ORT_D void occluded_lane(const SceneView &sv, const RenderHot &rv, const OccludedIO &io, const float4 *tab, uint32_t *lds_stack, const int tid,
                         const uint32_t lane_id, unsigned long long *pool) {
    uint32_t spill[kSpillStack];
    PathState P;
    HitState h;
    Trav T;
    Counters c;
    Prof pr;
    unsigned long long ray = 0;
    float bound = 0.0f;
    bool tracing = false, held = false, more = true;
    for (;;) {
        if (!tracing) {
            if (held) {
                h.runner_t = fminf(h.runner_t, bound);
                resolve_hit<COUNTERS, TABS, kLdsStack, kBlock, true>(sv, tab, P.org, P.dir, T.inv_d, lane_id, h, c, pr, lds_stack, spill, tid);
                io.out[ray] = (h.hit_mat != 0u && h.best_t < bound) ? (uint8_t)1 : (uint8_t)0;
                held = false;
            }
            if (more) {
                const unsigned long long j = pool ? draw_job(rv, pool) : ORT_NEXT_JOB(rv.c->next_job);
                if (j < rv.c->job_count) {
                    const float2 *r = io.q.rays + 3ull * j;
                    const float2 a = r[0], b = r[1], e = r[2];
                    const float tm = io.tmax ? io.tmax[j] : __builtin_inff();
                    P.org = mk(a.x, a.y, b.x);
                    P.dir = mk(b.y, e.x, e.y);
                    ray = j;
                    if (COUNTERS) c.rays++;
                    const bool forced = sv.force_fallback_mask != 0xffffffffu && (om_f32_bits(P.dir.x) & sv.force_fallback_mask) == 0u;
                    bound = (tm > 0.0f) ? fminf(tm, 3.402823466e+38f) : 0.0f;
// ... 110 lines not shown
```

offline_raytracer_amd/csrc/ort_plan.h:

```cpp
#ifndef ORT_PLAN_H
#define ORT_PLAN_H

#include <stddef.h>
#include <stdint.h>
#include <stdlib.h>
#include <string.h>

#include "../../include/ort.h"

namespace ort {

struct Knobs {
    uint32_t force_fallback_mask = 0xffffffffu;
    bool debug_util = false, debug_fallback = false, debug_drain = false;
    int cache_resident = -1;
    int refill_below = -1, descend_below = -1;
    bool wavefront = false;
    bool general_kernel = false;
    int lds_tables = -1;
    int exchange = -1;
    int long_min = -1, long_refill = -1, inflight_cap = -1, park_min = -1;
    int lpt = -1;
    int wide = -1;
    int waves5 = -1;
    int endgame_jobs = -1;
    int blocks_per_cu = -1;
    int job_batch = -1, batch_tail = -1;
};
inline int env_int(const char *name, int unset = -1) {
    const char *e = getenv(name);
    return e ? atoi(e) : unset;
}
inline Knobs read_knobs() {
    Knobs k;
    const char *e;
    if ((e = getenv("ORT_DEBUG_FORCE_FALLBACK"))) k.force_fallback_mask = (uint32_t)strtoul(e, nullptr, 0);
    k.debug_util = getenv("ORT_DEBUG_UTIL") != nullptr;
    k.debug_fallback = getenv("ORT_DEBUG_FALLBACK") != nullptr;
    k.debug_drain = getenv("ORT_DEBUG_DRAIN") != nullptr;
    k.cache_resident = env_int("ORT_CACHE_RESIDENT");
    k.refill_below = env_int("ORT_REFILL_BELOW");
    k.descend_below = env_int("ORT_DESCEND_BELOW");
    k.wavefront = (e = getenv("ORT_MODE")) && strcmp(e, "wavefront") == 0;
    k.general_kernel = (e = getenv("ORT_KERNEL")) && strcmp(e, "general") == 0;
    k.lds_tables = env_int("ORT_LDS_TABLES");
    k.exchange = env_int("ORT_EXCHANGE");
    k.long_min = env_int("ORT_LONG_MIN");
    k.long_refill = env_int("ORT_LONG_REFILL");
    k.inflight_cap = env_int("ORT_INFLIGHT_CAP");
    k.park_min = env_int("ORT_PARK_MIN");
    k.lpt = env_int("ORT_LPT");
    k.wide = env_int("ORT_WIDE");
    k.waves5 = env_int("ORT_WAVES5");
    k.endgame_jobs = env_int("ORT_ENDGAME_JOBS");
    k.blocks_per_cu = env_int("ORT_BLOCKS_PER_CU");
    k.job_batch = env_int("ORT_JOB_BATCH");
    k.batch_tail = env_int("ORT_BATCH_TAIL");
    return k;
}

constexpr uint32_t kPlanBlock = 256;
constexpr uint32_t kPlanLdsStack = 24;
constexpr uint32_t kPlanStashVecs = 9, kPlanCapL = 128, kPlanCapR = 192;
constexpr uint32_t kPlanTabPro = 1u, kPlanTabLights = 2u, kPlanTabMats = 8u;
constexpr uint32_t kPlanAllTabs = kPlanTabPro | kPlanTabLights | kPlanTabMats;
constexpr uint32_t kPlanTabMatCap = 48, kPlanTabLightCap = 64, kPlanTabProCap = 40;
enum : int { PLAN_JOBS_EXPLICIT = 0, PLAN_JOBS_PIXEL = 1, PLAN_JOBS_CHUNK = 2 };

inline unsigned int persistent_blocks(int cu_count, unsigned int per_cu) { return (unsigned int)(cu_count > 0 ? cu_count : 256) * per_cu; }
inline unsigned int upload_max_blocks(int cu_count, const Knobs &kn) {
    unsigned int per_cu = kn.blocks_per_cu > 0 ? (unsigned int)kn.blocks_per_cu : 4u;
    if (per_cu < 1u || per_cu > 8u) per_cu = 4u;
    return persistent_blocks(cu_count, per_cu);
}

inline bool tree_is_cache_resident(size_t fast_tree_bytes, int knob) {
    return knob >= 0 ? knob != 0 : fast_tree_bytes <= (size_t)(16u << 20);
}

struct BlockGrid { uint32_t blocks_w, block_x0, block_y0, my_blocks, shard_index, shard_count; };
inline BlockGrid block_grid_for(const ort_render_params *p) {
    BlockGrid g;
    g.shard_count = p->shard_count > 1 ? p->shard_count : 1;
    g.shard_index = p->shard_count > 1 ? p->shard_index : 0;
    g.blocks_w = (uint32_t)((p->width + 7) / 8);
    uint32_t total = g.blocks_w * (uint32_t)((p->height + 7) / 8);
    g.block_x0 = g.block_y0 = 0;
    if (g.shard_count == 1 && p->x1 > p->x0 && p->y1 > p->y0) {
        g.block_x0 = (uint32_t)(p->x0 / 8);
        g.block_y0 = (uint32_t)(p->y0 / 8);
        g.blocks_w = (uint32_t)((p->x1 + 7) / 8) - g.block_x0;
        total = g.blocks_w * ((uint32_t)((p->y1 + 7) / 8) - g.block_y0);
    }
    g.my_blocks = (total > g.shard_index) ? (total - g.shard_index + g.shard_count - 1) / g.shard_count : 0;
    return g;
}

inline uint64_t shard_block_count(const ort_render_params *p) { return block_grid_for(p).my_blocks; }

inline uint64_t render_workspace_bytes(const ort_render_params *p) {
    if (p->policy != ORT_POLICY_CHUNK || p->chunk == 0) return 0;
    uint64_t nch = p->spp / p->chunk;
    return nch * (uint64_t)block_grid_for(p).my_blocks * 64ull * 12ull;
}
inline uint64_t render_views_workspace_bytes(const ort_render_params *p, uint32_t view_count) { return (uint64_t)view_count * render_workspace_bytes(p); }

inline uint32_t table_fit_flags(size_t material_count, size_t light_count, uint32_t pro_boxes, uint32_t pro_spheres, uint32_t pro_cyls) {
    uint32_t flags = 0;
    if (2ull * pro_boxes + pro_spheres + 4ull * pro_cyls <= kPlanTabProCap) flags |= kPlanTabPro;
    if (light_count <= kPlanTabLightCap) flags |= kPlanTabLights;
    if (material_count <= kPlanTabMatCap) flags |= kPlanTabMats;
    return flags;
}

struct SceneTraits {
    bool diffuse_only = false;
    uint32_t tab_flags = 0;
    size_t fast_tree_bytes = 0;
    float sah_cost = 0;
    bool has_wide = false;
    int cu_count = 0;
    unsigned int max_blocks = 0;
};

inline void plan_loop_exits(bool cache_resident_tree, const Knobs &kn, int *refill_below, int *descend_below) {
    *refill_below = kn.refill_below >= 0 ? kn.refill_below : (cache_resident_tree ? 16 : 32);
    if (*refill_below < 1) *refill_below = 1;
    if (*refill_below > 64) *refill_below = 64;
    *descend_below = kn.descend_below >= 0 ? kn.descend_below : (cache_resident_tree ? 8 : 16);
    if (*descend_below < 0) *descend_below = 0;
    if (*descend_below > 64) *descend_below = 64;
}

inline void plan_job_batches(unsigned long long job_count, unsigned long long lanes, const Knobs &kn, uint32_t *job_batch, unsigned long long *batch_until) {
    *job_batch = kn.job_batch >= 0 ? (uint32_t)kn.job_batch : (job_count >= 96ull * lanes ? 128u : 64u);
    const unsigned long long per_lane = kn.batch_tail >= 0 ? (unsigned long long)kn.batch_tail : 8ull * ((*job_batch + 63u) / 64u);
    const unsigned long long tail = per_lane * lanes;
    *batch_until = job_count > tail ? job_count - tail : 0ull;
// ... 232 lines not shown
```

offline_raytracer_amd/csrc/ort_scene.h:

```cpp
#ifndef ORT_SCENE_H
#define ORT_SCENE_H

#include <math.h>
#include <stdint.h>
#include <algorithm>
#include <string>
#include <vector>

#include "../../include/ort.h"

namespace ort {

struct HostMesh {
    std::vector<float> vertices;
    std::vector<uint32_t> indices;
    uint32_t mat = 0;
    ort_v3 aabb_min = {0, 0, 0}, aabb_max = {0, 0, 0};
};

struct DevNode {
    float lo0[3], hi0[3], lo1[3], hi1[3];
    uint32_t child0, child1, pad0, pad1;
};
static_assert(sizeof(DevNode) == 64, "node record must be 64 B");
// ... 85 lines not shown
    std::vector<ort_sphere> spheres;
    std::vector<ort_box> boxes;
    std::vector<ort_cylinder> cylinders;
    std::vector<ort_light> lights;
    std::vector<HostMesh> meshes;
    ort_v3 ambient = {0, 0, 0};
    ort_v3 camera_p = {0, 0, 0};
    float camera_quat[4] = {0, 0, 0, 1};
    float camera_height_ratio = 0;
    int32_t screen_width = 0, screen_height = 0;

    bool reference_csg = false;

    Tree tree;
    RefTree ref;
    DeviceScene *dev = nullptr;
};

int parse_scn_text(const char *text, size_t size, const char *base_dir, Scene *scene, std::string *err);
int read_file(const char *path, std::vector<char> *out);
void camera_basis(const Scene &s, int32_t width, int32_t height, ort_camera *out);
void camera_from_pose(const ort_v3 &p, const float quat_xyzw[4], float height_ratio, int32_t width, int32_t height, ort_camera *out);

inline void scene_origin_box(const Scene &s, float lo[3], float hi[3]) {
    lo[0] = hi[0] = s.camera_p.x; lo[1] = hi[1] = s.camera_p.y; lo[2] = hi[2] = s.camera_p.z;
    auto grow = [&](float x, float y, float z, float r) {
        const float p[3] = {x, y, z};
        for (int k = 0; k < 3; ++k) { lo[k] = std::min(lo[k], p[k] - r); hi[k] = std::max(hi[k], p[k] + r); }
    };
    for (const ort_sphere &q : s.spheres) grow(q.center.x, q.center.y, q.center.z, fabsf(q.r));
    for (const ort_box &q : s.boxes) { grow(q.min.x, q.min.y, q.min.z, 0.0f); grow(q.max.x, q.max.y, q.max.z, 0.0f); }
    for (const ort_cylinder &q : s.cylinders) {
        grow(q.base.x, q.base.y, q.base.z, fabsf(q.r));
        grow(q.base.x + q.axis.x, q.base.y + q.axis.y, q.base.z + q.axis.z, fabsf(q.r));
    }
    for (const HostMesh &m : s.meshes)
        for (size_t i = 0; i + 2 < m.vertices.size(); i += 3) grow(m.vertices[i], m.vertices[i + 1], m.vertices[i + 2], 0.0f);
}

int build_tree(Scene *scene, std::string *err);
int build_ref_tree(Scene *scene, std::string *err);

uint32_t rgbe_pack(float r, float g, float b);

int device_count(int *n, std::string *err);
int device_upload(Scene *scene, int device, std::string *err);
void device_release(Scene *scene);
struct RenderCall {
    bool host;
    void *stream;
    ort_stats *stats;
    const ort_tile_job *jobs;
    uint32_t job_count;
    uint32_t *job_states;
    const ort_view *views;
    uint32_t view_count;
    const ort_adaptive *ad;
};
int device_render(Scene *scene, const ort_render_params *p, const RenderCall &c, void *out_rgb, void *out_spp, void *out_m2, void *states, std::string *err);
int device_unit_eval(int device, const void *records, uint32_t n, float *out, std::string *err);
struct QueryCall {
    bool host;
    uint64_t count;
    uint32_t flags;
    void *stream;
    ort_stats *stats;
};
int device_raycast(Scene *scene, const QueryCall &q, const void *rays, void *hits, std::string *err);
int device_occluded(Scene *scene, const QueryCall &q, const void *rays, const void *tmax, void *out, std::string *err);
int device_radiance(Scene *scene, const QueryCall &q, const void *rays, const void *seeds, uint32_t spp, float rr, const ort_adaptive *ad, void *out,
                    void *out_spp, void *out_m2, void *states, std::string *err);
struct Comm;
uint64_t comm_shard_blocks(int32_t w, int32_t h, uint32_t index, uint32_t count);
void pack_blocks_host(const float *full, int32_t w, int32_t h, uint32_t index, uint32_t count, float *packed);
void unpack_blocks_host(const float *packed, int32_t w, int32_t h, uint32_t index, uint32_t count, float *full);
int unpack_blocks_device(const void *d_packed, int32_t w, int32_t h, uint32_t index, uint32_t count, void *d_full, void *stream, std::string *err);
int comm_unique_id(void *id, std::string *err);
int comm_create(const void *id, int rank, int world, int device, Comm **out, std::string *err);
int comm_create_local(int world, const int *devices, Comm **out, std::string *err);
void comm_destroy(Comm *c);
int gather_framebuffer(Comm *c, const void *d_packed, void *d_full, int32_t w, int32_t h, void *stream, std::string *err);
int gather_framebuffer_local(Comm **cs, int world, const void *const *d_packed, void *d_full_root, int32_t w, int32_t h,
                             void *const *streams, std::string *err);
void cylinder_frame_for(const ort_cylinder &c, float rot[9], float *len);

}

struct ort_scene : public ort::Scene {};
struct ort_comm;

#endif
```

offline_raytracer_amd/csrc/ort_tree.cpp:

```cpp
#include <math.h>
#include <stdlib.h>
#include <string.h>

#include <algorithm>
#include <float.h>

#include "ort_scene.h"

namespace ort {

namespace {
constexpr float kPrologueBudget = 14.0f;

struct Box3 {
    float lo[3], hi[3];
    void reset() {
        for (int k = 0; k < 3; ++k) { lo[k] = FLT_MAX; hi[k] = -FLT_MAX; }
    }
    void grow(const Box3 &b) {
        for (int k = 0; k < 3; ++k) { lo[k] = std::min(lo[k], b.lo[k]); hi[k] = std::max(hi[k], b.hi[k]); }
    }
    void grow_point(const float p[3]) {
        for (int k = 0; k < 3; ++k) { lo[k] = std::min(lo[k], p[k]); hi[k] = std::max(hi[k], p[k]); }
    }
// ... 11 lines not shown
};

struct TriRef { uint32_t mesh, k; };

inline void v_sub(const float a[3], const float b[3], float r[3]) { r[0] = a[0] - b[0]; r[1] = a[1] - b[1]; r[2] = a[2] - b[2]; }
inline void v_cross(const float a[3], const float b[3], float r[3]) {
    r[0] = a[1] * b[2] - b[1] * a[2];
    r[1] = b[0] * a[2] - a[0] * b[2];
    r[2] = a[0] * b[1] - b[0] * a[1];
}
inline float v_len(const float a[3]) { return sqrtf(a[0] * a[0] + a[1] * a[1] + a[2] * a[2]); }
inline bool near0(float v) { return v >= -0.000001f && v < 0.000001f; }
inline bool v_is0(const float a[3]) { return near0(a[0]) && near0(a[1]) && near0(a[2]); }
inline void v_normalize(const float a[3], float r[3]) {
    float l = v_len(a);
    float diff = l - 0.0f;
    if (!(diff >= -0.000001f && diff < 0.000001f)) { r[0] = a[0] / l; r[1] = a[1] / l; r[2] = a[2] / l; }
    else { r[0] = r[1] = r[2] = 0.0f; }
}

void cylinder_frame(const ort_cylinder &c, float rot[9], float *len) {
    const float z[3] = {0, 0, 1}, x[3] = {1, 0, 0};
    float axis[3] = {c.axis.x, c.axis.y, c.axis.z};
    float id[9] = {1, 0, 0, 0, 1, 0, 0, 0, 1};
    memcpy(rot, id, sizeof(id));
    float cr[3];
    v_cross(axis, z, cr);
    if (!v_is0(cr)) {
        float a[3], b[3], t[3], cc[3];
        v_normalize(axis, a);
        v_cross(z, a, t);
        v_normalize(t, b);
        if (v_is0(b)) { v_cross(x, a, t); v_normalize(t, b); }
        v_cross(a, b, cc);
        memcpy(rot + 0, b, 12); memcpy(rot + 3, cc, 12); memcpy(rot + 6, a, 12);
    }
    *len = v_len(axis);
}

void pad_box(Box3 *b) {
    for (int k = 0; k < 3; ++k) {
        float m = std::max(fabsf(b->lo[k]), fabsf(b->hi[k]));
        float pad = 4e-7f * m + 1e-7f;
        b->lo[k] -= pad;
        b->hi[k] += pad;
    }
}

struct Builder {
    Scene *scene;
    std::vector<Prim> prims;
    std::vector<TriRef> tri_refs;
    Tree *tree;
    static constexpr int kBins = 16;
    uint32_t kMaxLeafTri = 4;
    uint32_t kMaxLeafOther = 2;
    static constexpr uint32_t kDepthBudget = kTreeDepthBudget;

    static constexpr float kNodeCost = 1.0f, kPrimCost = 1.2f;
    double sah_sum = 0;
    float root_area = 1;

    static uint32_t log2_ceil(uint32_t n) {
        uint32_t l = 0;
        while ((1u << l) < n) ++l;
        return l;
    }

    uint32_t emit_leaf(uint32_t begin, uint32_t end) {
        uint32_t kind = prims[begin].kind, count = end - begin, first = 0;
        switch (kind) {
        case PRIM_TRI:
            first = (uint32_t)tree->tris.size();
            for (uint32_t i = begin; i < end; ++i) {
                const TriRef &tr = tri_refs[prims[i].index];
                const HostMesh &m = scene->meshes[tr.mesh];
                const float *v0 = &m.vertices[3 * (size_t)m.indices[tr.k]];
                const float *v1 = &m.vertices[3 * (size_t)m.indices[tr.k + 1]];
                const float *v2 = &m.vertices[3 * (size_t)m.indices[tr.k + 2]];
                DevTri t;
                memcpy(t.v0, v0, 12);
                v_sub(v1, v0, t.e1);
                v_sub(v2, v0, t.e2);
                v_cross(t.e1, t.e2, t.n);
                tree->tri_slot[prims[i].index] = (uint32_t)tree->tris.size();
                tree->tris.push_back(t);
                tree->tri_mat.push_back(m.mat);
            }
            break;
        case PRIM_SPHERE:
            first = (uint32_t)tree->spheres.size();
            for (uint32_t i = begin; i < end; ++i) {
                const ort_sphere &s = scene->spheres[prims[i].index];
                tree->sphere_slot[prims[i].index] = (uint32_t)tree->spheres.size();
                tree->spheres.push_back(DevSphere{{s.center.x, s.center.y, s.center.z}, s.r});
                tree->sphere_mat.push_back(s.mat);
            }
            break;
        case PRIM_BOX:
            first = (uint32_t)tree->boxes.size();
            for (uint32_t i = begin; i < end; ++i) {
                const ort_box &b = scene->boxes[prims[i].index];
                tree->box_slot[prims[i].index] = (uint32_t)tree->boxes.size();
                tree->boxes.push_back(DevBox{{b.min.x, b.min.y, b.min.z}, 0, {b.max.x, b.max.y, b.max.z}, 0});
                tree->box_mat.push_back(b.mat);
            }
            break;
        default:
            first = (uint32_t)tree->cyls.size();
            for (uint32_t i = begin; i < end; ++i) {
                const ort_cylinder &c = scene->cylinders[prims[i].index];
                DevCyl d{};
                d.base[0] = c.base.x; d.base[1] = c.base.y; d.base[2] = c.base.z;
                d.r = c.r;
                cylinder_frame(c, d.rot, &d.len);
                tree->cyl_slot[prims[i].index] = (uint32_t)tree->cyls.size();
                tree->cyls.push_back(d);
                tree->cyl_mat.push_back(c.mat);
            }
            break;
        }
        tree->leaf_count++;
        tree->max_leaf_prims = std::max(tree->max_leaf_prims, count);
        return make_leaf(kind, first, count);
    }

    Box3 bounds(uint32_t begin, uint32_t end) const {
        Box3 b;
        b.reset();
        for (uint32_t i = begin; i < end; ++i) b.grow(prims[i].box);
        return b;
    }

    bool homogeneous(uint32_t begin, uint32_t end) const {
        for (uint32_t i = begin + 1; i < end; ++i)
            if (prims[i].kind != prims[begin].kind) return false;
        return true;
    }

    uint32_t build(uint32_t begin, uint32_t end, const Box3 &box, uint32_t depth) {
        tree->max_depth = std::max(tree->max_depth, depth);
        uint32_t count = end - begin;
        bool same_kind = homogeneous(begin, end);
        uint32_t max_leaf = (prims[begin].kind == PRIM_TRI) ? kMaxLeafTri : kMaxLeafOther;
        bool out_of_depth = depth >= kDepthBudget;
        if (same_kind && (count == 1 || (out_of_depth && count <= MAX_LEAF_PRIMS))) {
            sah_sum += (double)kPrimCost * count * box.half_area();
            return emit_leaf(begin, end);
        }

        uint32_t mid = begin;
        bool have_split = false;
        bool force_median = (depth + log2_ceil(count) + 2 >= kDepthBudget);
        if (!same_kind && count <= max_leaf) {
            uint32_t k0 = prims[begin].kind;
            mid = (uint32_t)(std::partition(prims.begin() + begin, prims.begin() + end,
                                            [&](const Prim &p) { return p.kind == k0; }) - prims.begin());
            have_split = (mid > begin && mid < end);
        }
        if (!have_split && !force_median) {
            Box3 cb;
            cb.reset();
            for (uint32_t i = begin; i < end; ++i) cb.grow_point(prims[i].centroid);
            float best_cost = FLT_MAX;
            int best_axis = -1, best_bin = -1;
            for (int axis = 0; axis < 3; ++axis) {
                float extent = cb.hi[axis] - cb.lo[axis];
// ... 12 lines not shown
                uint32_t right_n[kBins];
                Box3 acc;
                acc.reset();
                uint32_t n = 0;
                for (int b = kBins - 1; b > 0; --b) {
                    acc.grow(bin_box[b]);
                    n += bin_n[b];
                    right_area[b] = acc.half_area();
                    right_n[b] = n;
                }
                acc.reset();
                n = 0;
                for (int b = 0; b < kBins - 1; ++b) {
                    acc.grow(bin_box[b]);
                    n += bin_n[b];
                    if (n == 0 || right_n[b + 1] == 0) continue;
                    float cost = acc.half_area() * n + right_area[b + 1] * right_n[b + 1];
                    if (cost < best_cost) { best_cost = cost; best_axis = axis; best_bin = b; }
                }
            }
            if (best_axis >= 0) {
                float area = std::max(box.half_area(), 1e-30f);
                float split_cost = kNodeCost + kPrimCost * best_cost / area;
                float leaf_cost = kPrimCost * count;
                if (same_kind && count <= max_leaf && leaf_cost <= split_cost) {
                    sah_sum += (double)kPrimCost * count * box.half_area();
                    return emit_leaf(begin, end);
                }
                float lo = cb.lo[best_axis], scale = kBins / (cb.hi[best_axis] - cb.lo[best_axis]);
                mid = (uint32_t)(std::partition(prims.begin() + begin, prims.begin() + end, [&](const Prim &p) {
                          int b = (int)((p.centroid[best_axis] - lo) * scale);
                          b = std::max(0, std::min(kBins - 1, b));
                          return b <= best_bin;
                      }) - prims.begin());
                have_split = (mid > begin && mid < end);
            } else if (same_kind && count <= max_leaf) {
                sah_sum += (double)kPrimCost * count * box.half_area();
                return emit_leaf(begin, end);
            }
        }
        if (!have_split) {
            int axis = 0;
            float ext[3] = {box.hi[0] - box.lo[0], box.hi[1] - box.lo[1], box.hi[2] - box.lo[2]};
            if (ext[1] > ext[axis]) axis = 1;
            if (ext[2] > ext[axis]) axis = 2;
            mid = begin + count / 2;
            std::nth_element(prims.begin() + begin, prims.begin() + mid, prims.begin() + end,
                             [axis](const Prim &a, const Prim &b) { return a.centroid[axis] < b.centroid[axis]; });
        }

        uint32_t node_index = (uint32_t)tree->nodes.size();
        tree->nodes.push_back(DevNode{});
        sah_sum += (double)kNodeCost * box.half_area();
        Box3 lb = bounds(begin, mid), rb = bounds(mid, end);
        uint32_t c0 = build(begin, mid, lb, depth + 1);
        uint32_t c1 = build(mid, end, rb, depth + 1);
        DevNode &n = tree->nodes[node_index];
        memcpy(n.lo0, lb.lo, 12); memcpy(n.hi0, lb.hi, 12);
        memcpy(n.lo1, rb.lo, 12); memcpy(n.hi1, rb.hi, 12);
        n.child0 = c0; n.child1 = c1;
        return node_index | ((c0 | c1) & SPHERE_BELOW_BIT);
    }
};

}

DevMaterial make_dev_material(const ort_material &m) {
    DevMaterial d{};
    d.diffuse[0] = m.diffuse.x; d.diffuse[1] = m.diffuse.y; d.diffuse[2] = m.diffuse.z; d.ior = m.ior;
    d.specular[0] = m.specular[0]; d.specular[1] = m.specular[1]; d.specular[2] = m.specular[2];
    d.is_light = m.is_light ? 1u : 0u;
    d.transmission[0] = m.transmission.x; d.transmission[1] = m.transmission.y; d.transmission[2] = m.transmission.z;
    d.emit[0] = m.emit.x; d.emit[1] = m.emit.y; d.emit[2] = m.emit.z;
    float kd = v_len(d.diffuse), ks = v_len(d.specular), kt = v_len(d.transmission);
    float s = kd + ks + kt;
    d.pd_c = kd / s; d.ps_c = ks / s; d.pt_c = kt / s;
    const float pi_32 = 3.14159265358979323846264338327950288419716939937510582097494459230f;
    d.ed[0] = d.diffuse[0] / pi_32; d.ed[1] = d.diffuse[1] / pi_32; d.ed[2] = d.diffuse[2] / pi_32;
    return d;
}

void cylinder_frame_for(const ort_cylinder &c, float rot[9], float *len) { cylinder_frame(c, rot, len); }

static void renumber_top_levels(Tree *tree, uint32_t top) {
    const size_t n = tree->nodes.size();
    if (n <= 2) return;
    std::vector<uint32_t> order;
    std::vector<uint8_t> taken(n, 0);
    order.push_back(0);
    taken[0] = 1;
    for (size_t h = 0; h < order.size() && order.size() < top; ++h) {
        const DevNode &nd = tree->nodes[order[h]];
        const uint32_t ch[2] = {nd.child0, nd.child1};
        for (uint32_t c : ch) {
            if (c & LEAF_BIT) continue;
            const uint32_t i = c & NODE_INDEX_MASK;
            if (i < n && !taken[i] && order.size() < top) { taken[i] = 1; order.push_back(i); }
        }
    }
    for (uint32_t i = 0; i < n; ++i)
        if (!taken[i]) order.push_back(i);
    std::vector<uint32_t> new_of(n);
    for (uint32_t k = 0; k < n; ++k) new_of[order[k]] = k;
    std::vector<DevNode> out(n);
    for (uint32_t k = 0; k < n; ++k) {
        DevNode nd = tree->nodes[order[k]];
        if (!(nd.child0 & LEAF_BIT)) nd.child0 = (nd.child0 & ~NODE_INDEX_MASK) | new_of[nd.child0 & NODE_INDEX_MASK];
        if (!(nd.child1 & LEAF_BIT)) nd.child1 = (nd.child1 & ~NODE_INDEX_MASK) | new_of[nd.child1 & NODE_INDEX_MASK];
        out[k] = nd;
    }
    tree->nodes.swap(out);
}

static void collapse_to_wide(Tree *tree) {
    tree->nodes4.clear();
    tree->max_depth4 = 0;
    const std::vector<DevNode> &bn = tree->nodes;
    if (bn.empty()) return;
    struct Cand { uint32_t word; float lo[3], hi[3]; };
    auto area = [](const Cand &c) {
        const float dx = c.hi[0] - c.lo[0], dy = c.hi[1] - c.lo[1], dz = c.hi[2] - c.lo[2];
        return (dx < 0 || dy < 0 || dz < 0) ? 0.0f : dx * dy + dy * dz + dz * dx;
    };
    auto children_of = [&bn](uint32_t bi, Cand out[2]) {
        const DevNode &n = bn[bi];
        out[0].word = n.child0; memcpy(out[0].lo, n.lo0, 12); memcpy(out[0].hi, n.hi0, 12);
        out[1].word = n.child1; memcpy(out[1].lo, n.lo1, 12); memcpy(out[1].hi, n.hi1, 12);
    };
    struct Todo { uint32_t binary, wide, depth; };
    std::vector<Todo> queue;
    tree->nodes4.push_back(DevNode4{});
    queue.push_back(Todo{0u, 0u, 1u});
    for (size_t h = 0; h < queue.size(); ++h) {
        const Todo td = queue[h];
        tree->max_depth4 = std::max(tree->max_depth4, td.depth);
        Cand c[4];
        uint32_t n = 0;
        {
            Cand two[2];
            children_of(td.binary, two);
            for (int k = 0; k < 2; ++k)
                if (two[k].word != EMPTY_CHILD) c[n++] = two[k];
        }
        while (n < 4) {
            int pick = -1;
            float best = -1.0f;
            for (uint32_t k = 0; k < n; ++k)
                if (!(c[k].word & LEAF_BIT) && area(c[k]) > best) { best = area(c[k]); pick = (int)k; }
            if (pick < 0) break;
            Cand two[2];
            children_of(c[pick].word & NODE_INDEX_MASK, two);
            uint32_t live = 0;
            for (int k = 0; k < 2; ++k)
                if (two[k].word != EMPTY_CHILD) live++;
            if (n - 1 + live > 4) break;
            Cand next[4];
            uint32_t m = 0;
            for (uint32_t k = 0; k < n; ++k) {
                if ((int)k != pick) { next[m++] = c[k]; continue; }
                for (int j = 0; j < 2; ++j)
                    if (two[j].word != EMPTY_CHILD) next[m++] = two[j];
            }
            n = m;
            for (uint32_t k = 0; k < n; ++k) c[k] = next[k];
        }
        DevNode4 w{};
// ... 192 lines not shown
```

Measured before the change: 5206 Mpaths/s.

## Precompute unit triangle normals and tangent frames, fetch them with the hit winner

Triangle normals are now normalized on the host, and each triangle's tangent vector B is precomputed and stored in PrimInfo. The tangent words are streamed into LDS alongside chain/mat when the traversal winner is announced. The bounce path can then skip normalizing the hit normal and the tangent in sample_lobe. The change also uses finite-only AABB tests in the chain verdict and skips the modulo when there is a single light. The cost is a larger PrimInfo, two extra global-to-LDS loads per announce, and slight numeric differences from host-side normalization.

```diff
diff --git a/offline_raytracer_amd/csrc/ort_device.h b/offline_raytracer_amd/csrc/ort_device.h
--- a/offline_raytracer_amd/csrc/ort_device.h
+++ b/offline_raytracer_amd/csrc/ort_device.h
@@ -5,6 +5,7 @@
 #include <stdint.h>
 
 #include "ort_detmath.h"
+#include "ort_scene.h"
 
 namespace ortd {
 
@@ -273,6 +274,19 @@
     V3 C = cross(N, B);
     return add(add(scale(K.x, B), scale(K.y, C)), scale(K.z, N));
 }
+ORT_D V3 sample_lobe_n_tab(V3 N, float c, float cos_phi, float sin_phi, uint32_t wx, uint32_t wy) {
+    float s = __builtin_sqrtf(1.0f - c * c);
+    V3 K = mk(s * cos_phi, s * sin_phi, c);
+    if (absr(N.z - 1.0f) < 0.0001f) return K;
+    if (absr(N.z + 1.0f) < 0.0001f) return mk(K.x, -K.y, -K.z);
+    V3 B = mk(-N.y, N.x, 0);
+    if (wx != ort::kFrameIdentity) {
+        if (wx == ort::kFrameRuntime) B = normalize(B);
+        else B = mk(om_bits_f32(wx), om_bits_f32(wy), 0);
+    }
+    V3 C = cross(N, B);
+    return add(add(scale(K.x, B), scale(K.y, C)), scale(K.z, N));
+}
 ORT_D V3 sample_lobe(V3 N, float c, float phi) { return sample_lobe_n(normalize(N), c, ort_cosf(phi), ort_sinf(phi)); }
 
 struct BrdfDraw { float c, phi, choice; };
@@ -287,12 +301,13 @@
     else d.c = ort_cosf(ort_atan2f(rough * __builtin_sqrtf(e0), __builtin_sqrtf(1.0f - e0)));
     return d;
 }
-template <bool NORMALIZED = true, bool DIFFUSE_SCENE = false>
-ORT_D V3 sample_brdf_finish(V3 N, V3 Nn, V3 wo, const Mat &mt, BrdfDraw d, float cos_phi, float sin_phi, bool &is_trans) {
+template <bool NORMALIZED = true, bool DIFFUSE_SCENE = false, bool FRAME_TAB = false>
+ORT_D V3 sample_brdf_finish(V3 N, V3 Nn, V3 wo, const Mat &mt, BrdfDraw d, float cos_phi, float sin_phi, bool &is_trans, uint32_t wx = 0u, uint32_t wy = 0u) {
     float pd_c = mt.pd_c, ps_c = mt.ps_c;
     V3 wi;
     is_trans = false;
-    V3 m = sample_lobe_n(Nn, d.c, cos_phi, sin_phi);
+    V3 m = FRAME_TAB ? sample_lobe_n_tab(Nn, d.c, cos_phi, sin_phi, wx, wy)
+                     : sample_lobe_n(Nn, d.c, cos_phi, sin_phi);
     const bool diffuse_lobe = d.choice < pd_c;
     if (DIFFUSE_SCENE ? __builtin_expect(diffuse_lobe, 1) : diffuse_lobe) {
         wi = m;
diff --git a/offline_raytracer_amd/csrc/ort_kernels.hip b/offline_raytracer_amd/csrc/ort_kernels.hip
--- a/offline_raytracer_amd/csrc/ort_kernels.hip
+++ b/offline_raytracer_amd/csrc/ort_kernels.hip
@@ -73,6 +73,7 @@
     std::vector<float> view_tab_host;
     uint32_t tab_flags = 0;
     uint32_t light_count = 0;
+    bool frames = true;
     bool diffuse_only = false;
     DevBuf ref_nodes, ref_recs, chain_boxes;
     DevBuf tri_order, sphere_order, box_order, cyl_order;
@@ -129,18 +130,13 @@
     std::unique_ptr<DeviceScene> owner(new DeviceScene(device));
     DeviceScene *d = owner.get();
     const Tree &t = scene->tree;
+    d->knobs = read_knobs();
     if ((rc = upload_vec(t.nodes, &d->nodes, err))) return rc;
     if (!t.nodes4.empty() && 3u * t.max_depth4 <= (uint32_t)(kLdsStack - 4 + kSpillStack))
         if ((rc = upload_vec(t.nodes4, &d->nodes4, err))) return rc;
-    if ((rc = upload_vec(t.tris, &d->tris, err))) return rc;
     if ((rc = upload_vec(t.spheres, &d->spheres, err))) return rc;
     if ((rc = upload_vec(t.boxes, &d->boxes, err))) return rc;
     if ((rc = upload_vec(t.cyls, &d->cyls, err))) return rc;
-    {
-        std::vector<PrimInfo> info;
-        build_prim_info(t, scene->ref, info, d->info_box, d->info_cyl, d->info_sphere);
-        if ((rc = upload_vec(info, &d->prim_info, err))) return rc;
-    }
     const std::vector<DevMaterial> mats = dev_materials(*scene);
     if ((rc = upload_vec(mats, &d->materials, err))) return rc;
     d->diffuse_only = true;
@@ -150,6 +146,13 @@
         const float ks2 = dm.specular[0] * dm.specular[0] + dm.specular[1] * dm.specular[1] + dm.specular[2] * dm.specular[2];
         const float kt2 = dm.transmission[0] * dm.transmission[0] + dm.transmission[1] * dm.transmission[1] + dm.transmission[2] * dm.transmission[2];
         if (ks2 > 0.0f || kt2 > 0.0f || dm.ps_c > 0.0f || dm.pt_c > 0.0f) d->diffuse_only = false;
+    }
+    d->frames = d->knobs.frames != 0;
+    if ((rc = upload_vec(d->frames ? t.tris : raw_normal_tris(t), &d->tris, err))) return rc;
+    {
+        std::vector<PrimInfo> info;
+        build_prim_info(t, scene->ref, info, d->info_box, d->info_cyl, d->info_sphere, d->frames ? triangle_tangents(t) : std::vector<uint32_t>());
+        if ((rc = upload_vec(info, &d->prim_info, err))) return rc;
     }
     const std::vector<uint32_t> lis = light_sphere_flags(*scene);
     d->light_count = (uint32_t)lis.size();
@@ -175,7 +178,6 @@
     hipDeviceProp_t prop;
     ORT_HIP(hipGetDeviceProperties(&prop, device));
     d->cu_count = prop.multiProcessorCount;
-    d->knobs = read_knobs();
     d->max_blocks = upload_max_blocks(d->cu_count, d->knobs);
     d->bfs_queue_cap = (uint32_t)rt.nodes.size() + 8u;
     size_t fit = kBfsPoolBytes / ((size_t)d->bfs_queue_cap * sizeof(uint32_t));
@@ -367,6 +369,7 @@
     sv.chain_boxes = d->chain_boxes.as<const float4>();
     if (getenv("ORT_KNOBS_LIVE")) { const int keep = d->knobs.blocks_per_cu; d->knobs = read_knobs(); d->knobs.blocks_per_cu = keep; }
     sv.force_fallback_mask = d->knobs.force_fallback_mask;
+    sv.frames = d->frames ? 1u : 0u;
     sv.cold = (const ORT_CONSTANT_AS SceneCold *)d->cold.p;
     return sv;
 }
diff --git a/offline_raytracer_amd/csrc/ort_lane.h b/offline_raytracer_amd/csrc/ort_lane.h
--- a/offline_raytracer_amd/csrc/ort_lane.h
+++ b/offline_raytracer_amd/csrc/ort_lane.h
@@ -62,7 +62,7 @@
     unsigned long long *fallback_counters;
 };
 
-struct PrimInfo { uint32_t chain, mat; };
+struct PrimInfo { uint32_t chain, mat, bx, by; };
 
 struct SceneView {
     const float4 *tab_src;
@@ -83,20 +83,24 @@
     const ORT_CONSTANT_AS SceneCold *cold;
     unsigned long long *util;
     uint32_t force_fallback_mask;
+    uint32_t frames;
 };
 
-inline void build_prim_info(const Tree &t, const RefTree &rt, std::vector<PrimInfo> &out, uint32_t &info_box, uint32_t &info_cyl, uint32_t &info_sphere) {
+inline void build_prim_info(const Tree &t, const RefTree &rt, std::vector<PrimInfo> &out, uint32_t &info_box, uint32_t &info_cyl, uint32_t &info_sphere,
+                            const std::vector<uint32_t> &tangents = std::vector<uint32_t>()) {
     info_box = (uint32_t)t.tri_mat.size();
     info_cyl = info_box + (uint32_t)t.box_mat.size();
     info_sphere = info_cyl + (uint32_t)t.cyl_mat.size();
-    out.assign((size_t)info_sphere + t.sphere_mat.size(), PrimInfo{0u, 0u});
-    auto fill = [&out](uint32_t base, const std::vector<uint32_t> &chain, const std::vector<uint32_t> &mat) {
-        for (size_t i = 0; i < mat.size(); ++i) out[base + i] = PrimInfo{i < chain.size() ? chain[i] : 0u, mat[i]};
+    out.assign((size_t)info_sphere + t.sphere_mat.size(), PrimInfo{0u, 0u, kFrameRuntime, kFrameRuntime});
+    const bool tab = tangents.size() == 2u * t.tri_mat.size() && !tangents.empty();
+    auto fill = [&out](uint32_t base, const std::vector<uint32_t> &chain, const std::vector<uint32_t> &mat, uint32_t frame) {
+        for (size_t i = 0; i < mat.size(); ++i) out[base + i] = PrimInfo{i < chain.size() ? chain[i] : 0u, mat[i], frame, frame};
     };
-    fill(0u, rt.tri_chain, t.tri_mat);
-    fill(info_box, rt.box_chain, t.box_mat);
-    fill(info_cyl, rt.cyl_chain, t.cyl_mat);
-    fill(info_sphere, rt.sphere_chain, t.sphere_mat);
+    fill(0u, rt.tri_chain, t.tri_mat, kFrameRuntime);
+    if (tab) for (size_t i = 0; i < t.tri_mat.size(); ++i) { out[i].bx = tangents[2u * i]; out[i].by = tangents[2u * i + 1u]; }
+    fill(info_box, rt.box_chain, t.box_mat, tab ? kFrameIdentity : kFrameRuntime);
+    fill(info_cyl, rt.cyl_chain, t.cyl_mat, kFrameRuntime);
+    fill(info_sphere, rt.sphere_chain, t.sphere_mat, kFrameRuntime);
 }
 
 enum : int { JOBS_EXPLICIT = 0, JOBS_PIXEL = 1, JOBS_CHUNK = 2 };
@@ -308,17 +312,26 @@
     return slot + ((kind == PRIM_TRI) ? 0u : (kind == PRIM_BOX) ? sv.info_box : (kind == PRIM_CYL) ? sv.info_cyl : sv.info_sphere);
 }
 
-template <int BLOCK>
+template <int BLOCK, bool TANGENT = false>
 ORT_D void announce_winner(const SceneView &sv, uint32_t prim, uint32_t *lds_stack, int tid) {
     if (prim == kNoPrim) return;
     const PrimInfo *p = sv.prim_info + info_index(sv, prim);
 #ifdef ORT_HOST_SIM
     lds_stack[tid] = p->chain;
     lds_stack[BLOCK + tid] = p->mat;
+    if (TANGENT) { lds_stack[2 * BLOCK + tid] = p->bx; lds_stack[3 * BLOCK + tid] = p->by; }
 #else
     const uint32_t dst = (uint32_t)__builtin_amdgcn_readfirstlane((int)(uint32_t)(uintptr_t)(lds_stack + (tid & ~63)));
     const uint32_t *q = &p->mat;
     unsigned keep;
+    if (TANGENT) {
+        const uint32_t *qx = &p->bx, *qy = &p->by;
+        asm volatile("s_mov_b32 %0, m0\n\ts_mov_b32 m0, %5\n\ts_nop 0\n\tglobal_load_lds_dword %1, off\n\t"
+                     "s_add_u32 m0, %5, %6\n\ts_nop 0\n\tglobal_load_lds_dword %2, off\n\t"
+                     "s_add_u32 m0, %5, %7\n\ts_nop 0\n\tglobal_load_lds_dword %3, off\n\t"
+                     "s_add_u32 m0, %5, %8\n\ts_nop 0\n\tglobal_load_lds_dword %4, off\n\ts_mov_b32 m0, %0"
+                     : "=&s"(keep) : "v"(p), "v"(q), "v"(qx), "v"(qy), "s"(dst), "n"(BLOCK * 4), "n"(BLOCK * 8), "n"(BLOCK * 12) : "scc");
+    } else
     asm volatile("s_mov_b32 %0, m0\n\ts_mov_b32 m0, %3\n\ts_nop 0\n\tglobal_load_lds_dword %1, off\n\t"
                  "s_add_u32 m0, %3, %4\n\ts_nop 0\n\tglobal_load_lds_dword %2, off\n\ts_mov_b32 m0, %0"
                  : "=&s"(keep) : "v"(p), "v"(q), "s"(dst), "n"(BLOCK * 4) : "scc");
@@ -333,9 +346,10 @@
     chain = lds_stack[tid];
     mat = lds_stack[BLOCK + tid];
 }
+template <bool FINITE = false>
 ORT_D int ref_node_verdict(V3 lo, V3 hi, V3 org, V3 inv_d, float t_hit, float t_other, float &gap) {
     if ((org.x >= lo.x && org.x < hi.x) && (org.y >= lo.y && org.y < hi.y) && (org.z >= lo.z && org.z < hi.z)) return CH_ADMIT;
-    const float t = hit_aab_t(lo, hi, org, inv_d);
+    const float t = FINITE ? hit_aab_t_finite(lo, hi, org, inv_d) : hit_aab_t(lo, hi, org, inv_d);
     if (!(t >= kHitTMin)) return CH_REJECT;
     if (t <= t_hit || (t < t_other && t < t_hit * 1.0001f)) return CH_ADMIT;
     gap = fmaxf(gap, t);
@@ -379,8 +393,7 @@
     const uint32_t len = word >> 28, first = word & 0x07ffffffu;
     gap = 0.0f;
     if (len == 0u) return CH_ADMIT;
-    const bool finite = (om_f32_bits(inv_d.x) & 0x7fffffffu) < 0x7f800000u && (om_f32_bits(inv_d.y) & 0x7fffffffu) < 0x7f800000u &&
-                        (om_f32_bits(inv_d.z) & 0x7fffffffu) < 0x7f800000u;
+    const bool finite = all_finite6(org, inv_d);
     if (ORT_RARE(!(word & kChainNested) || !finite)) return chain_verdict_full(sv, first, len, org, inv_d, t_hit, t_other, gap);
     const float4 dlo = sv.chain_boxes[2u * first], dhi = sv.chain_boxes[2u * first + 1u];
     float4 jlo = dlo, jhi = dhi;
@@ -423,8 +436,8 @@
       g_cs[0][len]++; g_cs[1][jj < 0 ? 15 : jj]++; }
 #endif
     int verdict = CH_ADMIT;
-    if (found && !(hit_aab_t(mk(jlo.x, jlo.y, jlo.z), mk(jhi.x, jhi.y, jhi.z), org, inv_d) >= kHitTMin)) verdict = CH_REJECT;
-    else verdict = ref_node_verdict(mk(dlo.x, dlo.y, dlo.z), mk(dhi.x, dhi.y, dhi.z), org, inv_d, t_hit, t_other, gap);
+    if (found && !(hit_aab_t_finite(mk(jlo.x, jlo.y, jlo.z), mk(jhi.x, jhi.y, jhi.z), org, inv_d) >= kHitTMin)) verdict = CH_REJECT;
+    else verdict = ref_node_verdict<true>(mk(dlo.x, dlo.y, dlo.z), mk(dhi.x, dhi.y, dhi.z), org, inv_d, t_hit, t_other, gap);
 #if defined(ORT_HOST_SIM) && defined(ORT_CHAIN_CROSSCHECK)
     {
         float g2 = 0.0f;
@@ -512,6 +525,12 @@
     float runner_t = 0;
     uint32_t hit_mat = 0;
 };
+
+ORT_D V3 unit_hit_normal(const SceneView &sv, const HitState &h) {
+    const uint32_t kind = h.hit_prim >> 28;
+    if (!sv.frames || kind == PRIM_SPHERE || kind == PRIM_CYL) return normalize(h.hit_n);
+    return h.hit_n;
+}
 
 ORT_D size_t packed_index(const RenderHot &rv, uint32_t x, uint32_t y) {
     const uint32_t blk = ((y >> 3) - rv.c->block_y0) * rv.c->blocks_w + ((x >> 3) - rv.c->block_x0);
@@ -799,10 +818,11 @@
     return vm <= thr * thr;
 }
 
-template <bool COUNTERS, bool DIFFUSE = false, bool TABS = false, bool IMPLICIT = false, bool VIEWS = false, bool RAYS = false, bool ADAPT = false>
+template <bool COUNTERS, bool DIFFUSE = false, bool TABS = false, bool IMPLICIT = false, bool VIEWS = false, bool RAYS = false, bool ADAPT = false, bool FRAME_TAB = false>
 ORT_D bool produce_ray(const SceneView &sv, const RenderHot &rv, const float4 *tab, PathState &P, const HitState &h, Counters &c, Prof &pr,
                        float *focal_cache = nullptr, int focal_stride = 0, uint32_t spp_u = 0, uint32_t *late_flag = nullptr, bool no_new_job = false,
-                       unsigned long long *pool = nullptr, AdaptState *A = nullptr) {
+                       unsigned long long *pool = nullptr, AdaptState *A = nullptr,
+                       const uint32_t *frame_lds = nullptr ) {
     static_assert(!ADAPT || (IMPLICIT && (RAYS || VIEWS)), "the adaptive rule is built for the radiance queries and for one-pixel jobs of a batch of views");
     const V3 cam_p = mk(sv.cam[0], sv.cam[1], sv.cam[2]);
     const V3 cam_x = mk(sv.cam[3], sv.cam[4], sv.cam[5]);
@@ -823,8 +843,7 @@
         if (P.ps == PS_HIT) {
             bool alive = true;
             const uint32_t hit_mat = h.hit_mat;
-            n = normalize(h.hit_n);
-            ORT_SIM_RAY_HOOK((int)(P.pxy & 0xffffu), (int)(P.pxy >> 16), P.org, P.dir, h.best_t, n, hit_mat);
+            ORT_SIM_RAY_HOOK((int)(P.pxy & 0xffffu), (int)(P.pxy >> 16), P.org, P.dir, h.best_t, unit_hit_normal(sv, h), hit_mat);
             if (COUNTERS && P.primary) c.paths++;
             if (hit_mat) {
                 if (TABS) m = load_mat(tab + kTabMats, hit_mat);
@@ -840,6 +859,7 @@
                 }
                 alive = false;
             } else {
+                n = unit_hit_normal(sv, h);
                 if (P.primary) {
                     if (len2(m.kd) > 0.0f) P.weight = had(P.weight, m.kd);
                 } else {
@@ -863,7 +883,8 @@
             if (bounce) {
                 rng_step(P.rng);
                 if (sv.light_count) {
-                    uint32_t li = P.rng % sv.light_count;
+                    uint32_t li = 0u;
+                    if (sv.light_count != 1u) li = P.rng % sv.light_count;
                     uint32_t is_sphere;
                     if (TABS) is_sphere = ((const uint32_t *)tab)[4 * kTabLights + li];
                     else is_sphere = sv.light_is_sphere[li];
@@ -1042,6 +1063,12 @@
             ORT_PHASE(pr, sv, 2, true);
         }
         ORT_UTIL(sv, 7, true);
+#ifdef ORT_HOST_SIM
+        if constexpr (FRAME_TAB) if (bounce) {
+            const PrimInfo w = sv.prim_info[info_index(sv, h.hit_prim)];
+            if (w.bx != frame_lds[2 * kBlock] || w.by != frame_lds[3 * kBlock]) { fprintf(stderr, "the tangent words are not the final winner's\n"); abort(); }
+        }
+#endif
         float cs, sn;
         ort_sincosf(angle, &sn, &cs);
         if (DIFFUSE) {
@@ -1056,7 +1083,10 @@
             const V3 unit1 = normalize(bounce ? n : (RAYS ? ray_d : sub(focal, ap)));
             bool is_trans = false;
             V3 raw = unit1;
-            if (bounce) raw = sample_brdf_finish<false, true>(n, unit1, P.wo, m, draw, cs, sn, is_trans);
+            if (bounce) {
+                if constexpr (FRAME_TAB) raw = sample_brdf_finish<false, true, true>(n, unit1, P.wo, m, draw, cs, sn, is_trans, frame_lds[2 * kBlock], frame_lds[3 * kBlock]);
+                else raw = sample_brdf_finish<false, true>(n, unit1, P.wo, m, draw, cs, sn, is_trans);
+            }
             const V3 unit2 = normalize(raw);
             if (bounce) {
                 if (is_trans) P.org = add(P.org, scale(2.0f * kEps, P.dir));
@@ -1076,7 +1106,8 @@
             V3 raw, ap = mk(0, 0, 0);
             bool is_trans = false;
             if (bounce) {
-                raw = sample_brdf_finish<false>(n, normalize(n), P.wo, m, draw, cs, sn, is_trans);
+                if constexpr (FRAME_TAB) raw = sample_brdf_finish<false, false, true>(n, normalize(n), P.wo, m, draw, cs, sn, is_trans, frame_lds[2 * kBlock], frame_lds[3 * kBlock]);
+                else raw = sample_brdf_finish<false>(n, normalize(n), P.wo, m, draw, cs, sn, is_trans);
             } else {
                 if constexpr (RAYS) ap = ray_o;
                 else
@@ -1212,7 +1243,7 @@
     ORT_PHASE(pr, sv, 4, true);
 }
 
-template <bool COUNTERS, int LDS_ENTRIES, int BLOCK, bool TREELET = false, bool ANNOUNCE = false, bool WIDE = false>
+template <bool COUNTERS, int LDS_ENTRIES, int BLOCK, bool TREELET = false, int ANNOUNCE = 0 , bool WIDE = false>
 ORT_D bool traverse(const SceneView &sv, V3 org, V3 dir, Trav &T, HitState &h, uint32_t *lds_stack, uint32_t *spill, int tid,
                     int refill_below, int descend_below, Counters &c, Prof &pr, uint32_t excl = kNoPrim, const float4 *tab = nullptr) {
     bool tracing = true;
@@ -1263,7 +1294,7 @@
             }
             ORT_PHASE(pr, sv, 6, true);
         }
-        if (ANNOUNCE && !tracing) announce_winner<BLOCK>(sv, h.hit_prim, lds_stack, tid);
+        if (ANNOUNCE && !tracing) announce_winner<BLOCK, ANNOUNCE == 2>(sv, h.hit_prim, lds_stack, tid);
         if (refill_below > 0 && ORT_POPC64(ORT_BALLOT(tracing)) < refill_below) break;
     }
     T.cur = cur;
@@ -1271,7 +1302,7 @@
     return tracing;
 }
 
-template <bool COUNTERS, bool TABS, int LDS_ENTRIES, int BLOCK, bool ANNOUNCED = false, bool WIDE = false>
+template <bool COUNTERS, bool TABS, int LDS_ENTRIES, int BLOCK, bool ANNOUNCED = false, bool WIDE = false, bool FRAME_TAB = false>
 ORT_D void resolve_hit(const SceneView &sv, const float4 *tab, V3 org, V3 dir, V3 inv_d, uint32_t lane_id, HitState &h, Counters &c, Prof &pr,
                        uint32_t *lds_stack, uint32_t *spill, int tid) {
     uint32_t word = 0, mat = 0;
@@ -1326,7 +1357,12 @@
         }
     }
     recast_exactly<COUNTERS>(sv, recast, org, dir, inv_d, lane_id, h, c);
-    if (ORT_RARE(stale || recast)) mat = (h.hit_prim != kNoPrim) ? sv.prim_info[info_index(sv, h.hit_prim)].mat : 0u;
+    if (ORT_RARE(stale || recast)) {
+        PrimInfo pi = PrimInfo{0u, 0u, kFrameRuntime, kFrameRuntime};
+        if (h.hit_prim != kNoPrim) pi = sv.prim_info[info_index(sv, h.hit_prim)];
+        mat = pi.mat;
+        if (FRAME_TAB) { lds_stack[2 * BLOCK + tid] = pi.bx; lds_stack[3 * BLOCK + tid] = pi.by; }
+    }
     h.hit_mat = (h.hit_prim != kNoPrim) ? mat : 0u;
 }
 
@@ -1360,18 +1396,18 @@
             ORT_UTIL(sv, 3, true);
             ORT_UTIL(sv, 4, P.ps == PS_HIT);
             ORT_PHASE(pr, sv, 7, true);
-            if (P.ps == PS_HIT) resolve_hit<COUNTERS, TABS, kLdsStack, kBlock, true, WIDE>(sv, tab, P.org, P.dir, T.inv_d, lane_id, h, c, pr, lds_stack, spill, tid);
+            if (P.ps == PS_HIT) resolve_hit<COUNTERS, TABS, kLdsStack, kBlock, true, WIDE, true>(sv, tab, P.org, P.dir, T.inv_d, lane_id, h, c, pr, lds_stack, spill, tid);
             ORT_PHASE(pr, sv, 0, P.ps == PS_HIT);
-            if constexpr (ADAPT) tracing = produce_ray<COUNTERS, DIFFUSE, TABS, IMPLICIT, VIEWS, false, true>(sv, rv, tab, P, h, c, pr, lds_focal + tid, kBlock, spp_u, nullptr, false, pool, A);
+            if constexpr (ADAPT) tracing = produce_ray<COUNTERS, DIFFUSE, TABS, IMPLICIT, VIEWS, false, true, true>(sv, rv, tab, P, h, c, pr, lds_focal + tid, kBlock, spp_u, nullptr, false, pool, A, lds_stack + tid);
             else
-            tracing = produce_ray<COUNTERS, DIFFUSE, TABS, IMPLICIT, VIEWS>(sv, rv, tab, P, h, c, pr, lds_focal + tid, kBlock, spp_u, nullptr, false, pool);
+            tracing = produce_ray<COUNTERS, DIFFUSE, TABS, IMPLICIT, VIEWS, false, false, true>(sv, rv, tab, P, h, c, pr, lds_focal + tid, kBlock, spp_u, nullptr, false, pool, nullptr, lds_stack + tid);
             if (tracing) {
                 begin_ray<COUNTERS, TABS, kLdsStack, kBlock>(sv, tab, P, T, h, c, pr, lds_stack, spill, tid);
                 if (COUNTERS) c.rays++;
             }
         }
         if (ORT_BALLOT(P.ps != PS_DONE) == 0ull) break;
-        if (tracing) tracing = traverse<COUNTERS, kLdsStack, kBlock, TABS && !WIDE, true, WIDE>(sv, P.org, P.dir, T, h, lds_stack, spill, tid, rv.refill_below, rv.descend_below, c, pr, kNoPrim, tab);
+        if (tracing) tracing = traverse<COUNTERS, kLdsStack, kBlock, TABS && !WIDE, 2, WIDE>(sv, P.org, P.dir, T, h, lds_stack, spill, tid, rv.refill_below, rv.descend_below, c, pr, kNoPrim, tab);
     }
     flush_counters(rv, c, COUNTERS);
 }
@@ -1895,7 +1931,7 @@
             if (held) {
                 resolve_hit<COUNTERS, TABS, kLdsStack, kBlock, true>(sv, tab, P.org, P.dir, T.inv_d, lane_id, h, c, pr, lds_stack, spill, tid);
                 const uint32_t src = h.hit_prim != kNoPrim ? io.prim_src[info_index(sv, h.hit_prim)] : kNoPrim;
-                const V3 n = normalize(h.hit_n);
+                const V3 n = unit_hit_normal(sv, h);
                 uint2 *o = io.hits + 3ull * ray;
                 o[0] = make_uint2(om_f32_bits(h.best_t), om_f32_bits(n.x));
                 o[1] = make_uint2(om_f32_bits(n.y), om_f32_bits(n.z));
diff --git a/offline_raytracer_amd/csrc/ort_plan.h b/offline_raytracer_amd/csrc/ort_plan.h
--- a/offline_raytracer_amd/csrc/ort_plan.h
+++ b/offline_raytracer_amd/csrc/ort_plan.h
@@ -25,6 +25,7 @@
     int waves5 = -1;
     int endgame_jobs = -1;
     int blocks_per_cu = -1;
+    int frames = -1;
     int job_batch = -1, batch_tail = -1;
 };
 inline int env_int(const char *name, int unset = -1) {
@@ -54,6 +55,7 @@
     k.waves5 = env_int("ORT_WAVES5");
     k.endgame_jobs = env_int("ORT_ENDGAME_JOBS");
     k.blocks_per_cu = env_int("ORT_BLOCKS_PER_CU");
+    k.frames = env_int("ORT_FRAMES");
     k.job_batch = env_int("ORT_JOB_BATCH");
     k.batch_tail = env_int("ORT_BATCH_TAIL");
     return k;
diff --git a/offline_raytracer_amd/csrc/ort_scene.h b/offline_raytracer_amd/csrc/ort_scene.h
--- a/offline_raytracer_amd/csrc/ort_scene.h
+++ b/offline_raytracer_amd/csrc/ort_scene.h
@@ -191,6 +191,9 @@
 int gather_framebuffer(Comm *c, const void *d_packed, void *d_full, int32_t w, int32_t h, void *stream, std::string *err);
 int gather_framebuffer_local(Comm **cs, int world, const void *const *d_packed, void *d_full_root, int32_t w, int32_t h,
                              void *const *streams, std::string *err);
+std::vector<DevTri> raw_normal_tris(const Tree &t);
+constexpr uint32_t kFrameIdentity = 0x7fc00001u, kFrameRuntime = 0x7fc00002u;
+std::vector<uint32_t> triangle_tangents(const Tree &t);
 void cylinder_frame_for(const ort_cylinder &c, float rot[9], float *len);
 
 }
diff --git a/offline_raytracer_amd/csrc/ort_tree.cpp b/offline_raytracer_amd/csrc/ort_tree.cpp
--- a/offline_raytracer_amd/csrc/ort_tree.cpp
+++ b/offline_raytracer_amd/csrc/ort_tree.cpp
@@ -117,7 +117,9 @@
                 memcpy(t.v0, v0, 12);
                 v_sub(v1, v0, t.e1);
                 v_sub(v2, v0, t.e2);
-                v_cross(t.e1, t.e2, t.n);
+                float raw[3];
+                v_cross(t.e1, t.e2, raw);
+                v_normalize(raw, t.n);
                 tree->tri_slot[prims[i].index] = (uint32_t)tree->tris.size();
                 tree->tris.push_back(t);
                 tree->tri_mat.push_back(m.mat);
@@ -296,6 +298,30 @@
 
 void cylinder_frame_for(const ort_cylinder &c, float rot[9], float *len) { cylinder_frame(c, rot, len); }
 
+std::vector<uint32_t> triangle_tangents(const Tree &t) {
+    auto absr = [](float v) { if (v <= 0.0f) v *= -1.0f; return v; };
+    auto bits = [](float f) { uint32_t u; memcpy(&u, &f, 4); return u; };
+    std::vector<uint32_t> out(2u * t.tris.size(), 0u);
+    for (size_t i = 0; i < t.tris.size(); ++i) {
+        float N[3], B[3] = {0, 0, 0};
+        v_normalize(t.tris[i].n, N);
+        if (!(absr(N[2] - 1.0f) < 0.0001f) && !(absr(N[2] + 1.0f) < 0.0001f)) {
+            const float raw[3] = {-N[1], N[0], 0.0f};
+            v_normalize(raw, B);
+        }
+        const bool nan = B[0] != B[0] || B[1] != B[1];
+        out[2u * i] = nan ? kFrameRuntime : bits(B[0]);
+        out[2u * i + 1u] = nan ? kFrameRuntime : bits(B[1]);
+    }
+    return out;
+}
+
+std::vector<DevTri> raw_normal_tris(const Tree &t) {
+    std::vector<DevTri> out = t.tris;
+    for (DevTri &r : out) v_cross(r.e1, r.e2, r.n);
+    return out;
+}
+
 static void renumber_top_levels(Tree *tree, uint32_t top) {
     const size_t n = tree->nodes.size();
     if (n <= 2) return;
```

Result: faster. 5277 Mpaths/s (median of 6 runs) (+1.4%).
